# BOpermanis/SP-SLAM

Hardware: AMD Instinct MI355X
Metric: RGB-D frames/sec (track+planes+poseOpt) at 640x480; ATE vs CPU ref (higher is better)
Workload: dtype u8+f32+f64

## Files before the change

### include/spslam_gpu.h

```cpp
#ifndef SPSLAM_GPU_H
#define SPSLAM_GPU_H

#include <stddef.h>
#include <stdint.h>

#ifdef __cplusplus
extern "C" {
#endif

#define SPSLAM_OK 0
#define SPSLAM_ERR_ARG (-1)
#define SPSLAM_ERR_CAPACITY (-2)
#define SPSLAM_ERR_HIP (-3)
#define SPSLAM_ERR_NOT_READY (-4)

typedef struct spslam_ctx spslam_ctx;

typedef struct spslam_keypoint {
    float x, y;
    float size;
    float angle;
    float response;
    int32_t octave;
    int32_t class_id;
} spslam_keypoint;

typedef struct spslam_orb_params {
    int nfeatures;
    float scale_factor;
    int nlevels;
    int ini_th_fast;
    int min_th_fast;
    int width, height;
    int max_batch;
} spslam_orb_params;

#define SPSLAM_MAX_LEVELS 8

int spslam_create(int device, const spslam_orb_params* params, spslam_ctx** out);
void spslam_destroy(spslam_ctx* ctx);
const char* spslam_last_error(const spslam_ctx* ctx);

int spslam_orb_tables(const spslam_ctx* ctx, int* nlevels, float* scale, float* inv_scale, float* sigma2,
                      float* inv_sigma2, int* features_per_level);

int spslam_orb_max_keypoints(const spslam_ctx* ctx);

int spslam_orb_extract(spslam_ctx* ctx, const uint8_t* gray, int w, int h, int stride, spslam_keypoint* kps,
                       uint8_t* desc, int cap, int* n);

int spslam_orb_extract_batch_device(spslam_ctx* ctx, const uint8_t* d_gray, int n_frames, size_t frame_stride,
                                    int stride, spslam_keypoint* d_kps, uint8_t* d_desc, int* d_counts,
                                    int cap_per_frame, void* hip_stream);

int spslam_orb_debug_stage(spslam_ctx* ctx, int frame, int level, int stage, void* out, int cap, int* n);
int spslam_orb_level_size(const spslam_ctx* ctx, int level, int* w, int* h);

typedef struct spslam_point_obs {
    float u, v;
    float ur;
    float inv_sigma2;
    float xw[3];
    int32_t kp_index;
} spslam_point_obs;

#define SPSLAM_PLANE_EDGE 0
#define SPSLAM_PARALLEL_EDGE 1
#define SPSLAM_VERTICAL_EDGE 2

typedef struct spslam_plane_obs {
    float meas[4];
    float world[4];
    int32_t kind;
    int32_t plane_index;
    int32_t map_plane_id;
    int32_t pad;
} spslam_plane_obs;

typedef struct spslam_plane_config {
    double angle_info, distance_info, parallel_info, vertical_info, chi, vp_chi;
} spslam_plane_config;

typedef struct spslam_pose_problem {
    float Tcw[16];
    float fx, fy, cx, cy, bf;
    int32_t n_points;
    int32_t n_planes;
    int32_t point_offset;
    int32_t plane_offset;
    int32_t pad;
} spslam_pose_problem;

typedef struct spslam_pose_result {
    float Tcw[16];
    int32_t n_inliers;
    int32_t lm_iterations;
    int32_t trial_passes;
    int32_t trials;
} spslam_pose_result;

int spslam_pose_optimize(spslam_ctx* ctx, const spslam_pose_problem* problem, const spslam_point_obs* points,
                         const spslam_plane_obs* planes, const spslam_plane_config* cfg, spslam_pose_result* result,
                         uint8_t* point_outlier, uint8_t* plane_outlier);

int spslam_pose_optimize_batch_device(spslam_ctx* ctx, int n, const spslam_pose_problem* d_problems,
                                      const spslam_point_obs* d_points, const spslam_plane_obs* d_planes,
                                      const spslam_plane_config* cfg, const spslam_pose_result* d_init_from,
                                      spslam_pose_result* d_results, uint8_t* d_point_outlier,
                                      uint8_t* d_plane_outlier, void* hip_stream);

typedef struct spslam_lba_keyframe {
    float Tcw[16];
    float fx, fy, cx, cy, bf;
    int32_t id;
    int32_t fixed;
    int32_t pad;
} spslam_lba_keyframe;

typedef struct spslam_lba_point {
    float xw[3];
    int32_t id;
    int32_t obs_offset;
    int32_t n_obs;
} spslam_lba_point;

typedef struct spslam_lba_point_obs {
    int32_t kf;
    float u, v;
    float ur;
    float inv_sigma2;
} spslam_lba_point_obs;

typedef struct spslam_lba_plane {
    float world[4];
    int32_t id;
    int32_t obs_offset;
    int32_t n_obs;
    int32_t pad;
} spslam_lba_plane;

typedef struct spslam_lba_plane_obs {
    int32_t kf;
    int32_t kind;
    float meas[4];
} spslam_lba_plane_obs;

typedef struct spslam_lba_problem {
    int32_t n_kf, n_points, n_planes;
    int32_t kf_offset, point_offset, plane_offset;
    int32_t n_point_obs, n_plane_obs;
} spslam_lba_problem;

typedef struct spslam_lba_result {
    int32_t iterations[2];
    int32_t n_point_outliers;
    int32_t n_plane_outliers;
    int32_t status;
    int32_t trials;
    int32_t stopped;
    int32_t pad;
    float phase_us[8];
} spslam_lba_result;

int spslam_lba_optimize(spslam_ctx* ctx, const spslam_lba_problem* problem, const spslam_lba_keyframe* kfs,
                        const spslam_lba_point* points, const spslam_lba_point_obs* point_obs,
                        const spslam_lba_plane* planes, const spslam_lba_plane_obs* plane_obs,
                        const spslam_plane_config* cfg, float* kf_out, float* pt_out, float* pl_out,
                        uint8_t* point_obs_outlier, uint8_t* plane_obs_outlier, spslam_lba_result* result,
                        const volatile uint8_t* stop_flag);

#define SPSLAM_LBA_G2O_ORDER 0
#define SPSLAM_LBA_FAST_ORDER 1
int spslam_lba_set_order(spslam_ctx* ctx, int order);

int spslam_lba_debug_stop_after(spslam_ctx* ctx, int trials);

int spslam_lba_set_team(spslam_ctx* ctx, int workgroups);

int spslam_lba_optimize_batch_device(spslam_ctx* ctx, int n, const spslam_lba_problem* problems,
                                     const spslam_lba_problem* d_problems, const spslam_lba_keyframe* d_kfs,
                                     const spslam_lba_point* d_points, const spslam_lba_point_obs* d_point_obs,
                                     const spslam_lba_plane* d_planes, const spslam_lba_plane_obs* d_plane_obs,
                                     const spslam_plane_config* cfg, float* d_kf_out, float* d_pt_out,
                                     float* d_pl_out, uint8_t* d_point_obs_outlier, uint8_t* d_plane_obs_outlier,
                                     spslam_lba_result* d_results, const int32_t* d_stop_flags, void* hip_stream);

typedef struct spslam_plane_params {
    int cloud_dis;
    int min_size;
    float angle_threshold;
    float distance_threshold;
    float fx, fy, cx, cy;
    int width, height;
    double line_ratio;
    float line_distance_threshold;
    float image_bounds[4];
} spslam_plane_params;

typedef struct spslam_plane {
    float coef[4];
    int32_t n_inliers;
    int32_t inlier_offset;
    int32_t n_contour;
    int32_t contour_offset;
} spslam_plane;

int spslam_planes_configure(spslam_ctx* ctx, const spslam_plane_params* params);

int spslam_planes_capacity(const spslam_ctx* ctx, int* planes_cap, int* inlier_cap, int* contour_cap);

int spslam_planes_extract(spslam_ctx* ctx, const float* depth, int w, int h, int stride_floats,
                          spslam_plane* planes, int planes_cap, int* n_planes, int32_t* inliers, int32_t* contours);

int spslam_planes_extract_batch_device(spslam_ctx* ctx, const float* d_depth, int n_frames, size_t frame_stride,
                                       int stride_floats, spslam_plane* d_planes, int* d_counts,
                                       int32_t* d_inliers, int32_t* d_contours, void* hip_stream);

typedef struct spslam_supposed_plane {
    float coef[4];
    float line[6];
    int32_t source_plane;
    int32_t n_line;
    int32_t line_offset;
    int32_t n_patch;
    int32_t patch_offset;
    int32_t pad;
} spslam_supposed_plane;

int spslam_supposed_capacity(const spslam_ctx* ctx, int* supp_cap, int* line_cap, int* patch_points);

int spslam_planes_generate_from_boundaries(spslam_ctx* ctx, const float* depth, int w, int h, int stride_floats,
                                           spslam_supposed_plane* out, int cap, int* n, int32_t* line_idx,
                                           float* patch_xyz);

int spslam_planes_generate_from_boundaries_batch_device(spslam_ctx* ctx, const float* d_depth, int n_frames,
                                                        size_t frame_stride, int stride_floats,
                                                        const spslam_plane* d_planes, const int* d_counts,
                                                        const int32_t* d_contours, spslam_supposed_plane* d_out,
                                                        int* d_out_counts, int32_t* d_line_idx, float* d_patch,
                                                        void* hip_stream);

int spslam_planes_select_cloud_set(spslam_ctx* ctx, int set);

typedef struct spslam_line_candidate {
    float line[6];
    int32_t n_inliers;
    int32_t iterations;
    int32_t flags;
    int32_t idx_offset;
} spslam_line_candidate;
int spslam_supposed_debug(spslam_ctx* ctx, int frame, int plane, spslam_line_candidate* cand, int* n_cand,
                          int32_t* idx, int idx_cap);

int spslam_planes_debug(spslam_ctx* ctx, int frame, int what, void* out, int* n_points);

int spslam_debug_plane_labels(spslam_ctx* ctx, int keep);

int spslam_debug_plane_not_seen(spslam_ctx* ctx, const float* planes, int n_planes, const float* coefs, int n_coefs,
                                int* not_seen);

int spslam_debug_libm64(spslam_ctx* ctx, int kind, const double* a, const double* b, int n, double* out);

int spslam_debug_pose_spin_cap(spslam_ctx* ctx, int cap);

int spslam_debug_force_solve_failures(spslam_ctx* ctx, unsigned trial_mask);

#define SPSLAM_GRID_COLS 64
#define SPSLAM_GRID_ROWS 48

typedef struct spslam_frame_params {
    float fx, fy, cx, cy;
    float dist[5];
    float bf;
    int width, height;
} spslam_frame_params;

int spslam_frame_configure(spslam_ctx* ctx, const spslam_frame_params* params, float* bounds, float* grid_inv);

int spslam_frame_rgbd(spslam_ctx* ctx, const spslam_keypoint* kps, int n, const float* depth, int w, int h,
                      int stride_floats, spslam_keypoint* keys_un, float* mv_depth, float* mv_uright,
                      int32_t* grid_off, int32_t* grid_idx);

int spslam_frame_rgbd_batch_device(spslam_ctx* ctx, const spslam_keypoint* d_kps, const int* d_counts,
                                   int cap_per_frame, const float* d_depth, int n_frames, size_t frame_stride,
                                   int stride_floats, spslam_keypoint* d_keys_un, float* d_mv_depth,
                                   float* d_mv_uright, int32_t* d_grid_off, int32_t* d_grid_idx,
                                   int* d_plane_counts, int* d_supp_counts, void* hip_stream);

typedef struct spslam_map_plane {
    float world[4];
    int32_t id;
    int32_t boundary_offset;
    int32_t n_boundary;
    int32_t pad;
} spslam_map_plane;

typedef struct spslam_assoc_params {
    float dis_th;
    float angle_th;
    float ver_th;
    float par_th;
} spslam_assoc_params;

typedef struct spslam_assoc_frame {
    float Tcw[16];
    int32_t map_offset;
    int32_t n_map;
    int32_t carry;
    int32_t pad;
} spslam_assoc_frame;

int spslam_planes_associate(spslam_ctx* ctx, const spslam_assoc_frame* frame, const float* coefs, int n_planes,
                            const spslam_map_plane* map_planes, int n_map, const float* boundary_xyz,
                            int n_boundary, const spslam_assoc_params* params, int32_t* match, int32_t* parallel,
                            int32_t* vertical, int* new_plane);

int spslam_planes_associate_batch_device(spslam_ctx* ctx, int n_frames, const spslam_assoc_frame* d_frames,
                                         const void* d_planes_a, int stride_a, const int* d_count_a, int cap_a,
                                         const void* d_planes_b, int stride_b, const int* d_count_b, int cap_b,
                                         const spslam_map_plane* d_map, const float* d_boundary_xyz, int max_map,
                                         const spslam_assoc_params* params, int32_t* d_match, int32_t* d_parallel,
                                         int32_t* d_vertical, int* d_new_plane, void* hip_stream);

typedef struct spslam_proj_point {
    float xw[3];
    float angle;
    int32_t octave;
    int32_t n_obs;
    int32_t last_index;
    int32_t id;
    uint8_t desc[32];
} spslam_proj_point;

typedef struct spslam_proj_frame {
    float Tcw[16];
    float Tlw[16];
    int32_t point_offset;
    int32_t n_points;
    int32_t pad[2];
} spslam_proj_frame;

typedef struct spslam_match_params {
    float th;
    int32_t mono;
    int32_t check_orientation;
    int32_t retry_below;
} spslam_match_params;

int spslam_search_by_projection(spslam_ctx* ctx, const spslam_proj_frame* frame, const spslam_proj_point* points,
                                const spslam_keypoint* keys_un, const uint8_t* desc, const float* uright, int n_kp,
                                const int32_t* grid_off, const int32_t* grid_idx, const spslam_match_params* params,
                                int32_t* match, int* nmatches);

int spslam_search_by_projection_batch_device(spslam_ctx* ctx, int n_frames, const spslam_proj_frame* d_frames,
                                             const spslam_proj_point* d_points, int max_points,
                                             const spslam_keypoint* d_keys_un, const uint8_t* d_desc,
                                             const float* d_uright, const int32_t* d_grid_off,
                                             const int32_t* d_grid_idx, const int* d_counts, int cap,
                                             const spslam_match_params* params, int32_t* d_match, int* d_nmatches,
                                             void* hip_stream);

typedef struct spslam_local_point {
    float xw[3];
    float normal[3];
    float min_dist;
    float max_dist;
    int32_t id;
    int32_t n_obs;
    int32_t pad[2];
    uint8_t desc[32];
} spslam_local_point;

typedef struct spslam_local_frame {
    float Tcw[16];
    int32_t point_offset;
    int32_t n_points;
    int32_t seen_offset;
    int32_t stamp;
} spslam_local_frame;

typedef struct spslam_local_params {
    float th;
    float nn_ratio;
    float view_cos_limit;
    int32_t pad;
} spslam_local_params;

int spslam_search_local_points(spslam_ctx* ctx, const spslam_local_frame* frame, const spslam_local_point* points,
                               const spslam_keypoint* keys_un, const uint8_t* desc, const float* uright, int n_kp,
                               const int32_t* grid_off, const int32_t* grid_idx, const uint8_t* taken,
                               const spslam_local_params* params, int32_t* match, int* nmatches, uint8_t* in_view);

int spslam_search_local_points_batch_device(spslam_ctx* ctx, int n_frames, const spslam_local_frame* d_frames,
                                            const spslam_local_point* d_points, int max_points,
                                            const spslam_keypoint* d_keys_un, const uint8_t* d_desc,
                                            const float* d_uright, const int32_t* d_grid_off,
                                            const int32_t* d_grid_idx, const int* d_counts, int cap,
                                            const uint8_t* d_taken, const spslam_local_params* params,
                                            int32_t* d_match, int* d_nmatches, uint8_t* d_in_view,
                                            const int32_t* d_seen, void* hip_stream);

typedef struct spslam_grab_params {
    int32_t channels;
    int32_t rgb;
    int32_t depth_u16;
    float depth_scale;
} spslam_grab_params;

int spslam_grab_rgbd(spslam_ctx* ctx, const uint8_t* color, int color_stride, const void* depth, int depth_stride,
                     int w, int h, const spslam_grab_params* params, uint8_t* gray, float* depth_out);

int spslam_grab_rgbd_batch_device(spslam_ctx* ctx, int n_frames, const uint8_t* d_color, size_t color_frame_stride,
                                  int color_stride, const void* d_depth, size_t depth_frame_stride, int depth_stride,
                                  int w, int h, const spslam_grab_params* params, uint8_t* d_gray, float* d_depth_out,
                                  void* hip_stream);

int spslam_grab_fuse_cloud(spslam_ctx* ctx, int enable);

#define SPSLAM_TRACK_MOTION_MODEL 0
#define SPSLAM_TRACK_DISCARD 1
#define SPSLAM_TRACK_LOCAL_MAP 2
#define SPSLAM_TRACK_MOTION_PRIOR 3
#define SPSLAM_TRACK_LAST_FRAME 4

typedef struct spslam_track_batch {
    const spslam_keypoint* keys_un;
    const float* uright;
    const int* kp_counts;
    int32_t cap;
    const spslam_proj_frame* proj_frames;
    const spslam_proj_point* proj_points;
    const int32_t* proj_match;
    spslam_local_frame* local_frames;
    const spslam_local_point* local_points;
    const int32_t* local_match;
    uint8_t* taken;
    const void* planes_a;
    const void* planes_b;
    const int* count_a;
    const int* count_b;
    int32_t stride_a, stride_b, cap_a, cap_b;
    const spslam_map_plane* map;
    const int32_t* assoc_match;
    const int32_t* assoc_parallel;
    const int32_t* assoc_vertical;
    spslam_assoc_frame* assoc_frames_next;
    const uint8_t* plane_outlier;
    int32_t* next_match;
    int32_t* next_parallel;
    int32_t* next_vertical;
    spslam_assoc_frame* assoc_frames_first;
    int32_t* seen;
    spslam_proj_frame* next_frames;
    spslam_proj_point* next_points;
    float* velocity;
    const uint8_t* point_outlier_local;
    spslam_pose_problem* problems;
    spslam_point_obs* points;
    spslam_plane_obs* planes;
    int32_t* edge_of_kp;
    const spslam_pose_result* results;
    const uint8_t* point_outlier;
    float fx, fy, cx, cy, bf;
    int32_t pad;
} spslam_track_batch;

int spslam_track_graph_batch_device(spslam_ctx* ctx, int n_frames, int stage, const spslam_track_batch* batch,
                                    void* hip_stream);

#define SPSLAM_REFKF_PREPARE 0
#define SPSLAM_REFKF_SELECT 1

typedef struct spslam_refkf_batch {
    const int32_t* nmatches;
    uint8_t* fallback;
    int32_t* refkf_counts;
    const int32_t* bow_nmatches;
    const int32_t* bow_match;
    const int32_t* refkf_rows;
    const int32_t* refkf_index;
    int32_t rows_stride, pad;
    const int32_t* refkf_sets;
    const spslam_assoc_frame* assoc_frames;
    uint8_t* apply;
    int8_t* state;
    int32_t* refkf_match;
    spslam_proj_frame* refkf_frames;
    spslam_assoc_frame* refkf_assoc;
} spslam_refkf_batch;

int spslam_track_refkf_batch_device(spslam_ctx* ctx, int n_frames, int stage, const spslam_track_batch* mm,
                                    const spslam_refkf_batch* rk, void* hip_stream);

typedef struct spslam_refkf_vote {
    const int32_t* kf_base;
    const int32_t* kf_sets;
    int32_t ids_per_kf;
    int32_t n_kf;
    int32_t new_kf;
    int32_t pad;
    const int8_t* state;
    int32_t* refkf_index;
    int32_t* refkf_sets;
    int32_t* refkf_pairs;
} spslam_refkf_vote;

int spslam_track_refkf_vote_batch_device(spslam_ctx* ctx, int n_frames, const spslam_track_batch* mm,
                                         const spslam_refkf_vote* vote, void* hip_stream);

typedef struct spslam_frame_region {
    void* dst;
    const void* src;
    int64_t frame_bytes;
    int64_t dst_stride;
    int64_t src_stride;
} spslam_frame_region;

int spslam_masked_frame_copy_device(spslam_ctx* ctx, int n_frames, const uint8_t* flags, int n_regions,
                                    const spslam_frame_region* regions, void* hip_stream);

typedef struct spslam_bow_params {
    float nn_ratio;
    int32_t check_orientation;
} spslam_bow_params;

int spslam_bow_load_vocabulary(spslam_ctx* ctx, const char* text, size_t len, int* k, int* L, int* n_nodes,
                               int* n_words);

int spslam_bow_transform(spslam_ctx* ctx, const uint8_t* desc, int n, int levelsup, uint32_t* bow_words,
                         double* bow_values, int* n_bow, uint32_t* fv_nodes, int32_t* fv_start,
                         int32_t* fv_features, int* n_fv);

int spslam_bow_transform_batch_device(spslam_ctx* ctx, int n_frames, const uint8_t* d_desc, const int* d_counts,
                                      int cap, int levelsup, uint32_t* d_bow_words, double* d_bow_values,
                                      int* d_n_bow, uint32_t* d_fv_nodes, int32_t* d_fv_start,
                                      int32_t* d_fv_features, int* d_n_fv, void* hip_stream);

typedef struct spslam_bow_side {
    const uint8_t* desc;
    const spslam_keypoint* keys;
    const uint8_t* has_point;
    const int* counts;
    const uint32_t* fv_nodes;
    const int32_t* fv_start;
    const int32_t* fv_features;
    const int* n_fv;
    int32_t cap;
    int32_t pad;
} spslam_bow_side;

int spslam_search_by_bow(spslam_ctx* ctx, const uint8_t* kf_desc, const spslam_keypoint* kf_keys,
                         const uint8_t* kf_has_point, int kf_n, const uint32_t* kf_fv_nodes,
                         const int32_t* kf_fv_start, const int32_t* kf_fv_features, int kf_n_fv,
                         const uint8_t* f_desc, const spslam_keypoint* f_keys, int f_n, const uint32_t* f_fv_nodes,
                         const int32_t* f_fv_start, const int32_t* f_fv_features, int f_n_fv,
                         const spslam_bow_params* params, int32_t* match, int* nmatches);

int spslam_search_by_bow_batch_device(spslam_ctx* ctx, int n_pairs, const int32_t* d_pairs,
                                      const spslam_bow_side* keyframe, const spslam_bow_side* frame,
                                      const spslam_bow_params* params, int32_t* d_match, int* d_nmatches,
                                      void* hip_stream);

typedef struct spslam_step_config {
    int32_t n_frames, width, height, kp_cap;
    int32_t pipelined, tail_priority, orb_priority, planes_priority;
    spslam_grab_params grab;
    spslam_match_params match;
    spslam_local_params local;
    spslam_assoc_params assoc;
    spslam_plane_config pose;
    float fx, fy, cx, cy, bf;
    int32_t pad;
} spslam_step_config;

typedef struct spslam_step_frames {
    const uint8_t* color;
    size_t color_frame_stride;
    const void* depth;
    size_t depth_frame_stride;
    int32_t color_stride, depth_stride;
} spslam_step_frames;

typedef struct spslam_step_tracking {
    const spslam_proj_frame* proj_frames;
    const spslam_proj_point* proj_points;
    spslam_local_frame* local_frames;
    const spslam_local_point* local_points;
    const spslam_assoc_frame* assoc_frames1;
    spslam_assoc_frame* assoc_frames2;
    const spslam_map_plane* map;
    const float* boundary_xyz;
    int32_t max_proj_points, max_local_points, max_map, pad;
} spslam_step_tracking;

typedef struct spslam_step_set {
    uint8_t* gray;
    float* depth;
    spslam_keypoint* kps;
    uint8_t* desc;
    int* counts;
    spslam_plane* planes;
    int* plane_counts;
    int32_t* inliers;
    int32_t* contours;
    spslam_supposed_plane* supposed;
    int* supposed_counts;
    int32_t* lines;
    float* patch;
} spslam_step_set;

typedef struct spslam_step_tail {
    spslam_keypoint* keys_un;
    float* mv_depth;
    float* uright;
    int32_t* grid_off;
    int32_t* grid_idx;
    int32_t* match;
    int* nmatches;
    uint8_t* taken;
    int32_t* local_match;
    int* local_nmatches;
    int32_t* edge_of_kp;
    int32_t* assoc[2][3];
    int* new_plane[2];
    spslam_pose_problem* problems[2];
    spslam_point_obs* points[2];
    spslam_plane_obs* planes[2];
    uint8_t* point_outlier[2];
    uint8_t* plane_outlier[2];
    spslam_pose_result* results[2];
} spslam_step_tail;

typedef struct spslam_step spslam_step;
int spslam_step_create(spslam_ctx* ctx, const spslam_step_config* cfg, const spslam_step_set* sets ,
                       const spslam_step_tail* tail , spslam_step** out);
int spslam_step_buffers(const spslam_step* step, spslam_step_set* sets , spslam_step_tail* tail);
int spslam_step_prime(spslam_step* step, const spslam_step_frames* first);
int spslam_step_run(spslam_step* step, const spslam_step_frames* next, const spslam_step_tracking* tracking);
int spslam_step_sync(spslam_step* step);
void* spslam_step_stream(const spslam_step* step);
void spslam_step_destroy(spslam_step* step);

int spslam_set_timing(spslam_ctx* ctx, int enable);
int spslam_kernel_times(spslam_ctx* ctx, double* total_ms, long long* launches, int max_kinds);
const char* spslam_kernel_name(int kind);

#ifdef __cplusplus
}
#endif

#endif
```

### sp-slam_amd/csrc/capi_ctx.h

```cpp
#pragma once
#include <hip/hip_runtime.h>

#include <algorithm>
#include <cstdint>
#include <cstdio>
#include <cstdlib>
#include <initializer_list>
#include <string>
#include <vector>

#include "../../include/spslam_gpu.h"
#include "orb_launch.h"
#include "plane_launch.h"
#include "pose_launch.h"
#include "supposed_launch.h"
#include "frame_launch.h"
#include "lba_launch.h"
#include "assoc_launch.h"
#include "bow_launch.h"
#include "match_launch.h"
#include "track_launch.h"
#include "grab_launch.h"

using namespace spslam;

struct EventTimer : KernelTimer {
    struct Pair { int kind; hipEvent_t e0, e1; };
    std::vector<Pair> pending;
    std::vector<hipEvent_t> pool;
    double total_ms[kNumKernelKinds] = {};
    long long count[kNumKernelKinds] = {};
    hipEvent_t cur[kNumKernelKinds] = {};
    hipEvent_t get() {
        if (!pool.empty()) { hipEvent_t e = pool.back(); pool.pop_back(); return e; }
        hipEvent_t e = nullptr;
        (void)hipEventCreate(&e);
        return e;
    }
    void begin(int kind, hipStream_t s) override { cur[kind] = get(); (void)hipEventRecord(cur[kind], s); }
    void end(int kind, hipStream_t s) override {
        hipEvent_t e1 = get();
        (void)hipEventRecord(e1, s);
        pending.push_back(Pair{kind, cur[kind], e1});
    }
    void collect() {
        for (auto& p : pending) {
            float ms = 0.f;
            if (hipEventSynchronize(p.e1) == hipSuccess && hipEventElapsedTime(&ms, p.e0, p.e1) == hipSuccess) {
                total_ms[p.kind] += ms;
                count[p.kind] += 1;
            }
            pool.push_back(p.e0);
            pool.push_back(p.e1);
        }
        pending.clear();
    }
    void reset() { collect(); for (int k = 0; k < kNumKernelKinds; k++) { total_ms[k] = 0; count[k] = 0; } }
    ~EventTimer() override {
        for (auto& p : pending) { (void)hipEventDestroy(p.e0); (void)hipEventDestroy(p.e1); }
        for (auto e : pool) (void)hipEventDestroy(e);
    }
};

template <class T = uint8_t>
struct DevBuf {
    T* p = nullptr;
    size_t cap = 0;
    DevBuf() = default;
    DevBuf(const DevBuf&) = delete;
    DevBuf& operator=(const DevBuf&) = delete;
    ~DevBuf() { release(); }
    operator T*() const { return p; }
    void release() {
        if (p) (void)hipFree(p);
        p = nullptr;
        cap = 0;
    }
    hipError_t alloc(size_t bytes) {
        release();
        const hipError_t e = hipMalloc((void**)&p, bytes);
        if (e == hipSuccess) cap = bytes; else p = nullptr;
        return e;
    }
    hipError_t reserve(size_t bytes, hipStream_t s) {
        if (bytes <= cap) return hipSuccess;
        const hipError_t e = hipStreamSynchronize(s);
        return e != hipSuccess ? e : alloc(bytes);
    }
};

struct CtxStreams {
    hipStream_t stream = nullptr;
    hipStream_t orb_aux = nullptr;
    hipEvent_t orb_fork = nullptr, orb_join = nullptr;
    hipEvent_t lba_done = nullptr;
    int32_t* h_lba_stop = nullptr;
    int32_t* d_lba_stop = nullptr;
    CtxStreams() = default;
    CtxStreams(const CtxStreams&) = delete;
    CtxStreams& operator=(const CtxStreams&) = delete;
    ~CtxStreams() {
        if (lba_done) (void)hipEventDestroy(lba_done);
        if (h_lba_stop) (void)hipHostFree(h_lba_stop);
        if (orb_fork) (void)hipEventDestroy(orb_fork);
        if (orb_join) (void)hipEventDestroy(orb_join);
        if (orb_aux) (void)hipStreamDestroy(orb_aux);
        if (stream) (void)hipStreamDestroy(stream);
    }
};

struct spslam_ctx : CtxStreams {
    int device = 0;
    int num_cus = 256;
    spslam_orb_params p{};
    std::string err;
    std::vector<float> scale, inv_scale, sigma2, inv_sigma2;
    std::vector<int> nfeat;
    int umax[16]{};
    OrbGeom geom{};
    long long pyr_frame_stride = 0, blur_frame_stride = 0;
    int max_kp = 0;
    DevBuf<> d_pyr, d_blur, d_score;
    OrbBuffers b{};
    DevBuf<uint32_t> d_cand, d_keys;
    DevBuf<uint16_t> d_cand_cnt, d_keynode;
    DevBuf<LevelKp> d_lvl_kp;
    DevBuf<int> d_lvl_cnt;
    DevBuf<> d_in;
    DevBuf<spslam_keypoint> d_kps;
    DevBuf<> d_desc;
    DevBuf<int> d_cnt;
    const uint8_t* last_gray = nullptr;
    size_t last_frame_stride = 0;
    int last_stride = 0, last_frames = 0;
    EventTimer* timer = nullptr;
    DevBuf<> d_pose_scratch;
    bool planes_ready = false;
    PlaneGeom pg{};
    PlaneBuffers pb{};
    float* plane_cloud[2] = {nullptr, nullptr};
    int cloud_set = 0;
    struct CloudTag { const float* depth = nullptr; int n = 0; } cloud_tag[2];
    bool grab_cloud = [] { const char* e = getenv("SPSLAM_GRAB_CLOUD"); return e && e[0] == '1'; }();
    DevBuf<> d_plane_scratch;
    DevBuf<float> d_depth_in;
    DevBuf<spslam_plane> d_planes1;
    DevBuf<int> d_plane_cnt1;
    DevBuf<int32_t> d_inl1, d_con1;
    int plane_last_frames = 0;
    SuppParams sp{};
    SuppBuffers sb{};
    DevBuf<> d_supp_scratch;
    DevBuf<spslam_supposed_plane> d_supp1;
    DevBuf<int> d_supp_cnt1;
    DevBuf<int32_t> d_line1;
    DevBuf<float> d_patch1;
    int supp_last_frames = 0;
    bool frame_ready = false;
    FrameGeom fg{};
    DevBuf<> d_frame1;
    DevBuf<> d_lba_scratch;
    DevBuf<long long> d_lba_off;
    int lba_stop_after = -1;
    int lba_order = SPSLAM_LBA_G2O_ORDER;
    int lba_team = 0;
    DevBuf<int> d_lba_ctl;
    int pose_spin_cap = 0;
    unsigned solve_fail_mask = 0;
    DevBuf<> d_lba_stage;
    DevBuf<int2> d_lba_work;
    DevBuf<float> d_assoc_dist;
    DevBuf<> d_match_scratch;
    DevBuf<> d_vocab;
    VocabDev vocab{};
    DevBuf<> d_bow_scratch;
    DevBuf<> d_bow_stage;

    ~spslam_ctx() {
        if (lba_done) (void)hipEventSynchronize(lba_done);
        delete timer;
    }
};

inline int fail(spslam_ctx* c, int code, const char* fmt, const char* what = "") {
    if (c) {
        char buf[512];
        std::snprintf(buf, sizeof buf, fmt, what);
        c->err = buf;
    }
    return code;
}
#define HIP_CHECK(ctx, expr)                                                                  \
    do {                                                                                      \
        hipError_t e_ = (expr);                                                               \
        if (e_ != hipSuccess) return fail(ctx, SPSLAM_ERR_HIP, #expr ": %s", hipGetErrorString(e_)); \
    } while (0)

struct StageSlot {
    const void* src;
    size_t upload, bytes;
    StageSlot(const void* s, size_t up, size_t b) : src(s), upload(up), bytes(b) {}
    StageSlot(const void* s, size_t b) : StageSlot(s, b, b) {}
    StageSlot(size_t b) : StageSlot(nullptr, 0, b) {}
};

inline size_t stage_layout(const StageSlot* slots, int n, size_t* off) {
    size_t bytes = 0;
    for (int i = 0; i < n; i++) { off[i] = bytes; bytes += (slots[i].bytes + 255) / 256 * 256; }
    return bytes;
}

struct Stage {
    static constexpr int kMaxSlots = 18;
    spslam_ctx* c;
    uint8_t* q = nullptr;
    bool temporary = false;
    size_t off[kMaxSlots] = {};
    explicit Stage(spslam_ctx* ctx) : c(ctx) {}
    Stage(const Stage&) = delete;
    Stage& operator=(const Stage&) = delete;
    ~Stage() { if (temporary && q) (void)hipFreeAsync(q, c->stream); }
    int open(std::initializer_list<StageSlot> slots, DevBuf<>* persistent = nullptr, size_t grow = 1) {
        const int n = (int)slots.size();
        if (n > kMaxSlots) return fail(c, SPSLAM_ERR_ARG, "too many staging slots%s", "");
        const size_t bytes = stage_layout(slots.begin(), n, off);
        if (!persistent) {
            HIP_CHECK(c, hipMallocAsync((void**)&q, bytes, c->stream));
            temporary = true;
        } else {
            if (bytes > persistent->cap) HIP_CHECK(c, persistent->reserve(bytes * grow, c->stream));
            q = *persistent;
        }
        for (int i = 0; i < n; i++) {
            const StageSlot& s = slots.begin()[i];
            if (s.upload) HIP_CHECK(c, hipMemcpyAsync(q + off[i], s.src, s.upload, hipMemcpyHostToDevice, c->stream));
        }
        return SPSLAM_OK;
    }
    template <class T>
    T* slot(int i) const { return (T*)(q + off[i]); }
    int close() {
        uint8_t* t = temporary ? q : nullptr;
        q = nullptr;
        if (t) HIP_CHECK(c, hipFreeAsync(t, c->stream));
        return SPSLAM_OK;
    }
};
```

### sp-slam_amd/csrc/capi_planes.cpp

```cpp
#include "capi_ctx.h"

#include <cmath>
#include <cstring>
#include <random>

namespace {

hipError_t configure_supposed(spslam_ctx* c, const spslam_plane_params* p) {
    const PlaneGeom& g = c->pg;
    SuppParams& sp = c->sp;
    sp.line_ratio = p->line_ratio;
    const double T = (double)p->line_distance_threshold * (double)p->line_distance_threshold;
    float f = (float)T;
    while ((double)f >= T && f > 0.f) f = std::nextafter(f, 0.f);
    while ((double)std::nextafter(f, 1.f) < T) f = std::nextafter(f, 1.f);
    sp.sqr_th_f = f;
    const bool nob = p->image_bounds[0] == 0.f && p->image_bounds[1] == 0.f && p->image_bounds[2] == 0.f &&
                     p->image_bounds[3] == 0.f;
    sp.min_x = nob ? 0.f : p->image_bounds[0];
    sp.max_x = nob ? (float)p->width : p->image_bounds[1];
    sp.min_y = nob ? 0.f : p->image_bounds[2];
    sp.max_y = nob ? (float)p->height : p->image_bounds[3];
    sp.supp_cap = kMaxSuppPerFrame;
    sp.line_cap = g.contour_cap;
    int ns = 0;
    for (float v = -0.25f; v < 0.25f; v = (float)((double)v + 0.01)) {
        if (ns >= kMaxPatchSteps) return hipErrorInvalidValue;
        sp.steps[ns++] = v;
    }
    sp.n_steps = ns;
    const size_t F = (size_t)c->p.max_batch, CC = (size_t)g.contour_cap;
    SuppBuffers& b = c->sb;
    const size_t bytes = (size_t)kSuppRndTable * 4 +
                         F * kMaxPlanesPerFrame * kMaxLinesPerBoundary * sizeof(LineCand) +
                         F * kMaxPlanesPerFrame * sizeof(int) + F * CC * (4 + 16 + 4 + 1) +
                         F * kMaxPlanesPerFrame * 8 * sizeof(long long) + 9 * 256;
    hipError_t e = c->d_supp_scratch.alloc(bytes);
    if (e != hipSuccess) return e;
    uint8_t* q = c->d_supp_scratch;
    auto carve = [&](size_t n) { uint8_t* r = q; q += (n + 255) / 256 * 256; return r; };
    b.rnd = (const uint32_t*)carve((size_t)kSuppRndTable * 4);
    b.cand = (LineCand*)carve(F * kMaxPlanesPerFrame * kMaxLinesPerBoundary * sizeof(LineCand));
    b.n_cand = (int*)carve(F * kMaxPlanesPerFrame * sizeof(int));
    b.line_idx = (int32_t*)carve(F * CC * 4);
    b.big = (float4*)carve(F * CC * 16);
    b.big_sh = (int*)carve(F * CC * 4);
    b.big_flag = (uint8_t*)carve(F * CC);
    b.prof = (long long*)carve(F * kMaxPlanesPerFrame * 8 * sizeof(long long));
    e = hipMemset(b.prof, 0, F * kMaxPlanesPerFrame * 8 * sizeof(long long));
    if (e != hipSuccess) return e;
    std::vector<uint32_t> tab(kSuppRndTable);
    std::mt19937 mt(12345u);
    for (auto& v : tab) v = (uint32_t)mt() >> 1;
    e = hipMemcpy((void*)b.rnd, tab.data(), tab.size() * 4, hipMemcpyHostToDevice);
    if (e != hipSuccess) return e;
    const size_t patch = (size_t)sp.n_steps * sp.n_steps;
    if ((e = c->d_supp1.alloc(sp.supp_cap * sizeof(spslam_supposed_plane))) != hipSuccess) return e;
    if ((e = c->d_supp_cnt1.alloc(16)) != hipSuccess) return e;
    if ((e = c->d_line1.alloc(CC * 4)) != hipSuccess) return e;
    return c->d_patch1.alloc(sp.supp_cap * patch * 12);
}

}

extern "C" {

int spslam_planes_configure(spslam_ctx* c, const spslam_plane_params* p) {
    if (!c || !p) return SPSLAM_ERR_ARG;
    if (p->cloud_dis < 1 || p->width < 1 || p->height < 1 || p->fx == 0.f || p->fy == 0.f)
        return fail(c, SPSLAM_ERR_ARG, "bad plane parameters%s", "");
    HIP_CHECK(c, hipSetDevice(c->device));
    HIP_CHECK(c, hipStreamSynchronize(c->stream));
    PlaneGeom& g = c->pg;
    g.w = p->width;
    g.h = p->height;
    g.ds = p->cloud_dis;
    g.W = (int)std::ceil(p->width / (float)p->cloud_dis);
    g.H = (int)std::ceil(p->height / (float)p->cloud_dis);
    g.N = g.W * g.H;
    if (g.H > 512) return fail(c, SPSLAM_ERR_ARG, "organized cloud taller than 512 rows%s", "");
    if (g.N > 160000) return fail(c, SPSLAM_ERR_ARG, "organized cloud larger than the LDS state map%s", "");
    if (3 * 10 * g.W * 4 > 65536) return fail(c, SPSLAM_ERR_ARG, "organized cloud wider than the LDS row band%s", "");
    g.fx = p->fx; g.fy = p->fy; g.cx = p->cx; g.cy = p->cy;
    g.min_size = p->min_size;
    g.ang_cos = std::cos((float)(0.017453 * p->angle_threshold));
    g.dist_th = p->distance_threshold;
    g.inlier_cap = g.N;
    g.contour_cap = 4 * g.N;
    const long long N = g.N, F = c->p.max_batch, IWH = (long long)(g.W + 1) * (g.H + 1);
    PlaneBuffers& b = c->pb;
    c->planes_ready = false;
    c->plane_last_frames = c->supp_last_frames = 0;
    c->plane_cloud[0] = c->plane_cloud[1] = nullptr;
    c->sb = SuppBuffers{};
    const int keep_labels = b.keep_labels;
    b = PlaneBuffers{};
    b.keep_labels = keep_labels;
    const long long SH = wave_size(g.W, g.H);
    b.cloud_fs = 3 * N; b.wave_fs = SH; b.dist_fs = N; b.integral_fs = 6 * (IWH + g.W + 1); b.normal_fs = 3 * N; b.pd_fs = N;
    b.labels_fs = N; b.work_fs = 4 * N; b.grown_fs = N; b.maps_fs = 2 * N;
    const size_t bytes = F * (sizeof(float) * (2 * b.cloud_fs + b.wave_fs + b.dist_fs + b.normal_fs + b.pd_fs) +
                              sizeof(double) * b.integral_fs + sizeof(uint32_t) * b.labels_fs +
                              sizeof(int) * (b.work_fs + b.grown_fs) + b.maps_fs + 16 * sizeof(long long)) + 8192;
    HIP_CHECK(c, c->d_plane_scratch.alloc(bytes));
    uint8_t* q = c->d_plane_scratch;
    auto carve = [&](size_t n) { uint8_t* r = q; q += (n + 255) / 256 * 256; return r; };
    b.integral = (double*)carve(F * b.integral_fs * sizeof(double));
    c->plane_cloud[0] = (float*)carve(F * b.cloud_fs * 4);
    c->plane_cloud[1] = (float*)carve(F * b.cloud_fs * 4);
    b.cloud = c->plane_cloud[0];
    c->cloud_set = 0;
    c->cloud_tag[0] = c->cloud_tag[1] = {};
    b.wave = (float*)carve(F * b.wave_fs * 4);
    b.dist = (float*)carve(F * b.dist_fs * 4);
    b.normal = (float*)carve(F * b.normal_fs * 4);
    b.pd = (float*)carve(F * b.pd_fs * 4);
    b.labels = (uint32_t*)carve(F * b.labels_fs * 4);
    b.work = (int*)carve(F * b.work_fs * 4);
    b.grown = (int*)carve(F * b.grown_fs * 4);
    b.maps = (uint8_t*)carve(F * b.maps_fs);
    b.ts = (long long*)carve(F * 16 * sizeof(long long));
    HIP_CHECK(c, c->d_depth_in.alloc((size_t)g.w * g.h * sizeof(float)));
    HIP_CHECK(c, c->d_planes1.alloc(kMaxPlanesPerFrame * sizeof(spslam_plane)));
    HIP_CHECK(c, c->d_plane_cnt1.alloc(16));
    HIP_CHECK(c, c->d_inl1.alloc((size_t)g.inlier_cap * 4));
    HIP_CHECK(c, c->d_con1.alloc((size_t)g.contour_cap * 4));
    HIP_CHECK(c, configure_supposed(c, p));
    c->planes_ready = true;
    return SPSLAM_OK;
}

int spslam_planes_capacity(const spslam_ctx* c, int* planes_cap, int* inlier_cap, int* contour_cap) {
    if (!c || !c->planes_ready) return SPSLAM_ERR_NOT_READY;
    if (planes_cap) *planes_cap = kMaxPlanesPerFrame;
    if (inlier_cap) *inlier_cap = c->pg.inlier_cap;
    if (contour_cap) *contour_cap = c->pg.contour_cap;
    return SPSLAM_OK;
}

int spslam_planes_extract_batch_device(spslam_ctx* c, const float* d_depth, int n_frames, size_t frame_stride,
                                       int stride_floats, spslam_plane* d_planes, int* d_counts,
                                       int32_t* d_inliers, int32_t* d_contours, void* hip_stream) {
    if (!c) return SPSLAM_ERR_ARG;
    if (!c->planes_ready) return fail(c, SPSLAM_ERR_NOT_READY, "spslam_planes_configure not called%s", "");
    if (!d_depth || !d_planes || !d_counts || !d_inliers || !d_contours || n_frames < 1 ||
        n_frames > c->p.max_batch || stride_floats < c->pg.w)
        return fail(c, SPSLAM_ERR_ARG, "bad argument%s", " to spslam_planes_extract_batch_device");
    HIP_CHECK(c, hipSetDevice(c->device));
    hipStream_t s = (hipStream_t)hip_stream;
    auto& tag = c->cloud_tag[c->cloud_set];
    const bool have_cloud = tag.depth == d_depth && n_frames <= tag.n &&
                            frame_stride == (size_t)c->pg.w * c->pg.h && stride_floats == c->pg.w;
    tag = {};
    HIP_CHECK(c, plane_launch(c->pg, c->pb, n_frames, d_depth, (long long)frame_stride, stride_floats, d_planes,
                              d_counts, kMaxPlanesPerFrame, d_inliers, d_contours, s, c->timer, have_cloud));
    c->plane_last_frames = n_frames;
    return SPSLAM_OK;
}

int spslam_planes_extract(spslam_ctx* c, const float* depth, int w, int h, int stride_floats, spslam_plane* planes,
                          int planes_cap, int* n_planes, int32_t* inliers, int32_t* contours) {
    if (!c || !n_planes) return SPSLAM_ERR_ARG;
    if (!c->planes_ready) return fail(c, SPSLAM_ERR_NOT_READY, "spslam_planes_configure not called%s", "");
    if (!depth || w != c->pg.w || h != c->pg.h || stride_floats < w)
        return fail(c, SPSLAM_ERR_ARG, "depth size does not match the plane configuration%s", "");
    HIP_CHECK(c, hipSetDevice(c->device));
    HIP_CHECK(c, hipMemcpy2DAsync(c->d_depth_in, (size_t)w * 4, depth, (size_t)stride_floats * 4, (size_t)w * 4, h,
                                  hipMemcpyHostToDevice, c->stream));
    int rc = spslam_planes_extract_batch_device(c, c->d_depth_in, 1, (size_t)w * h, w, c->d_planes1, c->d_plane_cnt1,
                                                c->d_inl1, c->d_con1, c->stream);
    if (rc) return rc;
    int n = 0;
    spslam_plane tmp[kMaxPlanesPerFrame];
    HIP_CHECK(c, hipMemcpyAsync(&n, c->d_plane_cnt1, sizeof(int), hipMemcpyDeviceToHost, c->stream));
    HIP_CHECK(c, hipMemcpyAsync(tmp, c->d_planes1, sizeof tmp, hipMemcpyDeviceToHost, c->stream));
    HIP_CHECK(c, hipStreamSynchronize(c->stream));
    *n_planes = n;
    if (n > planes_cap) return fail(c, SPSLAM_ERR_CAPACITY, "plane buffer too small%s", "");
    int ni = 0, nc = 0;
    for (int k = 0; k < n; k++) {
        planes[k] = tmp[k];
        ni = std::max(ni, tmp[k].inlier_offset + tmp[k].n_inliers);
        nc = std::max(nc, tmp[k].contour_offset + tmp[k].n_contour);
    }
    if (inliers && ni) HIP_CHECK(c, hipMemcpy(inliers, c->d_inl1, (size_t)ni * 4, hipMemcpyDeviceToHost));
    if (contours && nc) HIP_CHECK(c, hipMemcpy(contours, c->d_con1, (size_t)nc * 4, hipMemcpyDeviceToHost));
    return SPSLAM_OK;
}

int spslam_supposed_capacity(const spslam_ctx* c, int* supp_cap, int* line_cap, int* patch_points) {
    if (!c || !c->planes_ready) return SPSLAM_ERR_NOT_READY;
    if (supp_cap) *supp_cap = c->sp.supp_cap;
    if (line_cap) *line_cap = c->sp.line_cap;
    if (patch_points) *patch_points = c->sp.n_steps * c->sp.n_steps;
    return SPSLAM_OK;
}

int spslam_planes_select_cloud_set(spslam_ctx* c, int set) {
    if (!c) return SPSLAM_ERR_ARG;
    if (!c->planes_ready) return fail(c, SPSLAM_ERR_NOT_READY, "spslam_planes_configure not called%s", "");
    if (set < 0 || set > 1) return fail(c, SPSLAM_ERR_ARG, "cloud set not 0 or 1%s", "");
    c->pb.cloud = c->plane_cloud[set];
    c->cloud_set = set;
    return SPSLAM_OK;
}

int spslam_planes_generate_from_boundaries_batch_device(spslam_ctx* c, const float* d_depth, int n_frames,
                                                        size_t frame_stride, int stride_floats,
                                                        const spslam_plane* d_planes, const int* d_counts,
                                                        const int32_t* d_contours, spslam_supposed_plane* d_out,
                                                        int* d_out_counts, int32_t* d_line_idx, float* d_patch,
                                                        void* hip_stream) {
    if (!c) return SPSLAM_ERR_ARG;
    if (!c->planes_ready) return fail(c, SPSLAM_ERR_NOT_READY, "spslam_planes_configure not called%s", "");
    if (!d_depth || !d_planes || !d_counts || !d_contours || !d_out || !d_out_counts || !d_line_idx || !d_patch ||
        n_frames < 1 || stride_floats < c->pg.w)
        return fail(c, SPSLAM_ERR_ARG, "bad argument%s", " to spslam_planes_generate_from_boundaries_batch_device");
    if (n_frames > c->plane_last_frames)
        return fail(c, SPSLAM_ERR_NOT_READY, "%s", "more frames than the last plane extraction holds");
    HIP_CHECK(c, hipSetDevice(c->device));
    hipStream_t s = (hipStream_t)hip_stream;
    HIP_CHECK(c, supp_launch(c->pg, c->pb, c->sp, c->sb, n_frames, d_depth, (long long)frame_stride, stride_floats,
                             d_planes, d_counts, d_contours, d_out, d_out_counts, d_line_idx, d_patch, s, c->timer));
    c->supp_last_frames = n_frames;
    return SPSLAM_OK;
}

int spslam_planes_generate_from_boundaries(spslam_ctx* c, const float* depth, int w, int h, int stride_floats,
                                           spslam_supposed_plane* out, int cap, int* n, int32_t* line_idx,
                                           float* patch_xyz) {
    if (!c || !n) return SPSLAM_ERR_ARG;
    if (!c->planes_ready) return fail(c, SPSLAM_ERR_NOT_READY, "spslam_planes_configure not called%s", "");
    if (!depth || w != c->pg.w || h != c->pg.h || stride_floats < w)
        return fail(c, SPSLAM_ERR_ARG, "depth size does not match the plane configuration%s", "");
    if (c->plane_last_frames < 1) return fail(c, SPSLAM_ERR_NOT_READY, "%s", "spslam_planes_extract not called");
    HIP_CHECK(c, hipSetDevice(c->device));
    HIP_CHECK(c, hipMemcpy2DAsync(c->d_depth_in, (size_t)w * 4, depth, (size_t)stride_floats * 4, (size_t)w * 4, h,
                                  hipMemcpyHostToDevice, c->stream));
    int rc = spslam_planes_generate_from_boundaries_batch_device(c, c->d_depth_in, 1, (size_t)w * h, w, c->d_planes1,
                                                                 c->d_plane_cnt1, c->d_con1, c->d_supp1,
                                                                 c->d_supp_cnt1, c->d_line1, c->d_patch1, c->stream);
    if (rc) return rc;
    int m = 0;
    std::vector<spslam_supposed_plane> tmp(c->sp.supp_cap);
    HIP_CHECK(c, hipMemcpyAsync(&m, c->d_supp_cnt1, sizeof(int), hipMemcpyDeviceToHost, c->stream));
    HIP_CHECK(c, hipMemcpyAsync(tmp.data(), c->d_supp1, tmp.size() * sizeof(spslam_supposed_plane),
                                hipMemcpyDeviceToHost, c->stream));
    HIP_CHECK(c, hipStreamSynchronize(c->stream));
    *n = m;
    const int stored = std::min(m, c->sp.supp_cap);
    if (m > cap || m > c->sp.supp_cap) return fail(c, SPSLAM_ERR_CAPACITY, "supposed-plane buffer too small%s", "");
    int nl = 0;
    for (int k = 0; k < stored; k++) {
        out[k] = tmp[k];
        nl = std::max(nl, tmp[k].line_offset + tmp[k].n_line);
    }
    const size_t patch = (size_t)c->sp.n_steps * c->sp.n_steps;
    if (line_idx && nl) HIP_CHECK(c, hipMemcpy(line_idx, c->d_line1, (size_t)nl * 4, hipMemcpyDeviceToHost));
    if (patch_xyz && stored)
        HIP_CHECK(c, hipMemcpy(patch_xyz, c->d_patch1, stored * patch * 12, hipMemcpyDeviceToHost));
    return SPSLAM_OK;
}

int spslam_planes_associate_batch_device(spslam_ctx* c, int n_frames, const spslam_assoc_frame* d_frames,
                                         const void* d_planes_a, int stride_a, const int* d_count_a, int cap_a,
                                         const void* d_planes_b, int stride_b, const int* d_count_b, int cap_b,
                                         const spslam_map_plane* d_map, const float* d_boundary_xyz, int max_map,
                                         const spslam_assoc_params* params, int32_t* d_match, int32_t* d_parallel,
                                         int32_t* d_vertical, int* d_new_plane, void* hip_stream) {
    if (!c) return SPSLAM_ERR_ARG;
    if (n_frames < 1 || !d_frames || !params || !d_match || !d_parallel || !d_vertical || max_map < 0 ||
        (cap_a > 0 && (!d_planes_a || !d_count_a || stride_a < 16)) || cap_a < 0 || cap_b < 0 ||
        (cap_b > 0 && (!d_planes_b || !d_count_b || stride_b < 16)) || (max_map > 0 && (!d_map || !d_boundary_xyz)))
        return fail(c, SPSLAM_ERR_ARG, "bad argument%s", " to spslam_planes_associate_batch_device");
    HIP_CHECK(c, hipSetDevice(c->device));
    hipStream_t s = (hipStream_t)hip_stream;
    const size_t need = std::max<size_t>((size_t)n_frames * (cap_a + cap_b) * max_map * sizeof(float), 256);
    HIP_CHECK(c, c->d_assoc_dist.reserve(need, s));
    AssocSources S{(const uint8_t*)d_planes_a, cap_b > 0 ? (const uint8_t*)d_planes_b : nullptr, stride_a,
                   stride_b, d_count_a, cap_b > 0 ? d_count_b : nullptr, cap_a, cap_b};
    HIP_CHECK(c, assoc_launch(n_frames, d_frames, S, d_map, d_boundary_xyz, max_map, *params, c->d_assoc_dist,
                              d_match, d_parallel, d_vertical, d_new_plane, s, c->timer));
    return SPSLAM_OK;
}

int spslam_planes_associate(spslam_ctx* c, const spslam_assoc_frame* frame, const float* coefs, int n_planes,
                            const spslam_map_plane* map_planes, int n_map, const float* boundary_xyz,
                            int n_boundary, const spslam_assoc_params* params, int32_t* match, int32_t* parallel,
                            int32_t* vertical, int* new_plane) {
    if (!c || !frame || !params || n_planes < 0 || n_map < 0 || n_boundary < 0 ||
        (n_planes && (!coefs || !match || !parallel || !vertical)) || (n_map && !map_planes) ||
        (n_boundary && !boundary_xyz))
        return SPSLAM_ERR_ARG;
    for (int j = 0; j < n_map; j++)
        if (map_planes[j].n_boundary < 0 || map_planes[j].boundary_offset < 0 ||
            (long long)map_planes[j].boundary_offset + map_planes[j].n_boundary > n_boundary)
            return fail(c, SPSLAM_ERR_ARG, "map plane boundary range outside the boundary array%s", "");
    HIP_CHECK(c, hipSetDevice(c->device));
    spslam_assoc_frame F = *frame;
    F.map_offset = 0;
    F.n_map = n_map;
    const int cap = std::max(n_planes, 1);
    Stage st(c);
    if (int rc = st.open({{&F, sizeof F}, {coefs, (size_t)n_planes * 16, (size_t)cap * 16}, {&n_planes, sizeof(int)},
                           {map_planes, n_map * sizeof(spslam_map_plane), std::max(n_map, 1) * sizeof(spslam_map_plane)},
                           {boundary_xyz, (size_t)n_boundary * 12, (size_t)std::max(n_boundary, 1) * 12},
                           (size_t)cap * 4 * 3, sizeof(int)}))
        return rc;
    auto* d_out = st.slot<int32_t>(5);
    if (F.carry && n_planes) {
        HIP_CHECK(c, hipMemcpyAsync(d_out, match, (size_t)n_planes * 4, hipMemcpyHostToDevice, c->stream));
        HIP_CHECK(c, hipMemcpyAsync(d_out + cap, parallel, (size_t)n_planes * 4, hipMemcpyHostToDevice, c->stream));
        HIP_CHECK(c, hipMemcpyAsync(d_out + 2 * cap, vertical, (size_t)n_planes * 4, hipMemcpyHostToDevice, c->stream));
    }
    int rc = spslam_planes_associate_batch_device(
        c, 1, st.slot<spslam_assoc_frame>(0), st.slot<void>(1), 16, st.slot<int>(2), cap, nullptr, 0, nullptr, 0,
        st.slot<spslam_map_plane>(3), st.slot<float>(4), n_map, params, d_out, d_out + cap, d_out + 2 * cap,
        st.slot<int>(6), c->stream);
    if (rc) return rc;
    int np = 0;
    if (n_planes) {
        HIP_CHECK(c, hipMemcpyAsync(match, d_out, (size_t)n_planes * 4, hipMemcpyDeviceToHost, c->stream));
        HIP_CHECK(c, hipMemcpyAsync(parallel, d_out + cap, (size_t)n_planes * 4, hipMemcpyDeviceToHost, c->stream));
        HIP_CHECK(c, hipMemcpyAsync(vertical, d_out + 2 * cap, (size_t)n_planes * 4, hipMemcpyDeviceToHost, c->stream));
    }
    HIP_CHECK(c, hipMemcpyAsync(&np, st.slot<int>(6), sizeof(int), hipMemcpyDeviceToHost, c->stream));
    if ((rc = st.close())) return rc;
    HIP_CHECK(c, hipStreamSynchronize(c->stream));
    if (new_plane) *new_plane = np;
    return SPSLAM_OK;
}

int spslam_debug_plane_not_seen(spslam_ctx* c, const float* planes, int n_planes, const float* coefs, int n_coefs,
                                int* not_seen) {
    if (!c || n_planes < 0 || n_coefs < 0 || (n_planes && !planes) || (n_coefs && (!coefs || !not_seen)))
        return SPSLAM_ERR_ARG;
    if (!n_coefs) return SPSLAM_OK;
    HIP_CHECK(c, hipSetDevice(c->device));
    const size_t cb = (size_t)n_coefs * 16;
    Stage st(c);
    if (int rc = st.open({{planes, (size_t)n_planes * 16, (size_t)std::max(n_planes, 1) * 16}, {coefs, cb},
                          (size_t)n_coefs * 4}))
        return rc;
    HIP_CHECK(c, plane_not_seen_debug_launch(st.slot<float>(0), n_planes, st.slot<float>(1), n_coefs,
                                             st.slot<int>(2), c->stream));
    HIP_CHECK(c, hipMemcpyAsync(not_seen, st.slot<int>(2), (size_t)n_coefs * 4, hipMemcpyDeviceToHost, c->stream));
    if (int rc = st.close()) return rc;
    HIP_CHECK(c, hipStreamSynchronize(c->stream));
    return SPSLAM_OK;
}

int spslam_debug_plane_labels(spslam_ctx* c, int keep) {
    if (!c) return SPSLAM_ERR_ARG;
    c->pb.keep_labels = keep ? 1 : 0;
    return SPSLAM_OK;
}

int spslam_supposed_debug(spslam_ctx* c, int frame, int plane, spslam_line_candidate* cand, int* n_cand,
                          int32_t* idx, int idx_cap) {
    static_assert(sizeof(spslam_line_candidate) == sizeof(LineCand), "candidate layout");
    if (!c || !cand || !n_cand) return SPSLAM_ERR_ARG;
    if (frame < 0 || frame >= c->supp_last_frames || plane < 0 || plane >= kMaxPlanesPerFrame)
        return fail(c, SPSLAM_ERR_NOT_READY, "no supposed-plane data for that frame%s", "");
    HIP_CHECK(c, hipSetDevice(c->device));
    HIP_CHECK(c, hipDeviceSynchronize());
    int nc = 0;
    HIP_CHECK(c, hipMemcpy(&nc, c->sb.n_cand + frame * kMaxPlanesPerFrame + plane, sizeof(int), hipMemcpyDeviceToHost));
    nc = std::min(std::max(nc, 0), kMaxLinesPerBoundary);
    LineCand lc[kMaxLinesPerBoundary];
    if (nc)
        HIP_CHECK(c, hipMemcpy(lc, c->sb.cand + ((size_t)frame * kMaxPlanesPerFrame + plane) * kMaxLinesPerBoundary,
                               nc * sizeof(LineCand), hipMemcpyDeviceToHost));
    *n_cand = nc;
    int lo = 0;
    for (int k = 0; k < nc; k++) {
        std::memcpy(&cand[k], &lc[k], sizeof(LineCand));
        if (lc[k].flags & 1) {
            const int m = lc[k].n_inliers;
            if (idx && lo + m <= idx_cap && m)
                HIP_CHECK(c, hipMemcpy(idx + lo, c->sb.line_idx + (size_t)frame * c->pg.contour_cap + lc[k].idx_off,
                                       (size_t)m * 4, hipMemcpyDeviceToHost));
            cand[k].idx_offset = lo;
            lo += m;
        } else {
            cand[k].idx_offset = -1;
        }
    }
    return lo > idx_cap ? SPSLAM_ERR_CAPACITY : SPSLAM_OK;
}

int spslam_planes_debug(spslam_ctx* c, int frame, int what, void* out, int* n_points) {
    if (!c || !out) return SPSLAM_ERR_ARG;
    if (!c->planes_ready || frame < 0 || frame >= c->plane_last_frames)
        return fail(c, SPSLAM_ERR_NOT_READY, "no plane data for that frame%s", "");
    HIP_CHECK(c, hipSetDevice(c->device));
    HIP_CHECK(c, hipDeviceSynchronize());
    const PlaneBuffers& b = c->pb;
    const long long N = c->pg.N;
    if (n_points) *n_points = (int)N;
    if (what == 0 || what == 1) {
        const float* src = what == 0 ? b.cloud + frame * b.cloud_fs : b.normal + frame * b.normal_fs;
        std::vector<float> soa(3 * N);
        HIP_CHECK(c, hipMemcpy(soa.data(), src, 3 * N * 4, hipMemcpyDeviceToHost));
        float* o = (float*)out;
        for (long long i = 0; i < N; i++) { o[3 * i] = soa[i]; o[3 * i + 1] = soa[N + i]; o[3 * i + 2] = soa[2 * N + i]; }
        return SPSLAM_OK;
    }
    if (what == 2) {
        HIP_CHECK(c, hipMemcpy(out, b.dist + frame * b.dist_fs, N * 4, hipMemcpyDeviceToHost));
        return SPSLAM_OK;
    }
    if (what == 3) {
        bool in_lds = false;
        plane_segment_lds_bytes(c->pg, &in_lds);
        if (in_lds && !b.keep_labels)
            return fail(c, SPSLAM_ERR_NOT_READY, "labels are kept only after spslam_debug_plane_labels(ctx, 1)%s", "");
        HIP_CHECK(c, hipMemcpy(out, b.labels + frame * b.labels_fs, N * 4, hipMemcpyDeviceToHost));
        return SPSLAM_OK;
    }
    if (what == 4) {
        HIP_CHECK(c, hipMemcpy(out, b.ts + frame * 16, 16 * sizeof(long long), hipMemcpyDeviceToHost));
        return SPSLAM_OK;
    }
    if (what == 5) {
        HIP_CHECK(c, hipMemcpy(out, c->sb.prof + (size_t)frame * kMaxPlanesPerFrame * 8,
                               kMaxPlanesPerFrame * 8 * sizeof(long long), hipMemcpyDeviceToHost));
        return SPSLAM_OK;
    }
    return fail(c, SPSLAM_ERR_ARG, "unknown debug stage%s", "");
}

}
```

### sp-slam_amd/csrc/supposed_kernels.hip

```cpp
#include <cfloat>

#include "libm_restated.h"
#include "plane_not_seen.h"
#include "supposed_launch.h"

namespace spslam {
namespace supp {

constexpr int kThreads = 256, kWaves = 4;
constexpr int kMaxWaves = 8;
constexpr int kBatch = 64;
constexpr int kLdsPts = 2048;
constexpr int kMaxTrials = 1001;

#ifdef SPSLAM_SUPP_PROF
#define SUPP_CLK() ((long long)__builtin_amdgcn_s_memrealtime())
#define SUPP_T(k) do { if (t == 0) { const long long c_ = SUPP_CLK(); pr[k] += c_ - pt; pt = c_; } } while (0)
#else
#define SUPP_T(k) do { } while (0)
#endif

struct Shared {
    int s0[kBatch], s1[kBatch], cnt[kBatch];
    int nb, fail, done, have;
    int iterations, best, best_s0, best_s1;
    double k;
    float line[6];
    float acc[9];
    int red[kMaxWaves];
    int n_inl, flags;
    int s0x[kBatch], s1x[kBatch], nbb[2], failb[2];
};

__device__ __forceinline__ int wave_sum(int v) {
#pragma unroll
    for (int o = 32; o > 0; o >>= 1) v += __shfl_xor(v, o);
    return v;
}
template <int NT>
__device__ int block_sum(int v, Shared& S) {
    const int lane = threadIdx.x & 63, wave = threadIdx.x >> 6;
    v = wave_sum(v);
    __syncthreads();
    if (lane == 0) S.red[wave] = v;
    __syncthreads();
    int s = 0;
#pragma unroll
    for (int w = 0; w < NT / 64; w++) s += S.red[w];
    return s;
}

__device__ __forceinline__ void line_from_samples(const float4 a, const float4 b, float* c) {
    c[0] = a.x; c[1] = a.y; c[2] = a.z;
    float d0 = b.x - a.x, d1 = b.y - a.y, d2 = b.z - a.z;
    const float sq = d0 * d0 + d1 * d1 + d2 * d2;
    if (sq > 0.f) {
        const float s = sqrtf(sq);
        d0 /= s; d1 /= s; d2 /= s;
    }
    c[3] = d0; c[4] = d1; c[5] = d2;
}
__device__ __forceinline__ void normalize4(float* d) {
    const float sq = (d[0] * d[0] + d[2] * d[2]) + (d[1] * d[1] + 0.f);
    if (sq > 0.f) {
        const float s = sqrtf(sq);
        d[0] /= s; d[1] /= s; d[2] /= s;
    }
}
__device__ __forceinline__ float line_sqd(const float* lp, const float* ld, const float4 p) {
    const float ax = lp[0] - p.x, ay = lp[1] - p.y, az = lp[2] - p.z;
    const float cx = ay * ld[2] - az * ld[1];
    const float cy = az * ld[0] - ax * ld[2];
    const float cz = ax * ld[1] - ay * ld[0];
    return (cx * cx + cz * cz) + (cy * cy + 0.f);
}

__device__ void roots2(float b, float c, float* r) {
    r[0] = 0.f;
    float d = (float)(b * b - 4.0 * c);
    if (d < 0.0) d = 0.0;
    const float sd = sqrtf(d);
    r[2] = 0.5f * (b + sd);
    r[1] = 0.5f * (b - sd);
}
__device__ void roots3(const float (&m)[3][3], float* r) {
    const float c0 = m[0][0] * m[1][1] * m[2][2] + 2.f * m[0][1] * m[0][2] * m[1][2] - m[0][0] * m[1][2] * m[1][2] -
                     m[1][1] * m[0][2] * m[0][2] - m[2][2] * m[0][1] * m[0][1];
    const float c1 = m[0][0] * m[1][1] - m[0][1] * m[0][1] + m[0][0] * m[2][2] - m[0][2] * m[0][2] +
                     m[1][1] * m[2][2] - m[1][2] * m[1][2];
    const float c2 = m[0][0] + m[1][1] + m[2][2];
    if (fabsf(c0) < FLT_EPSILON) { roots2(c2, c1, r); return; }
    const float s_inv3 = (float)(1.0 / 3.0), s_sqrt3 = sqrtf(3.0f);
    const float c2_over_3 = c2 * s_inv3;
    float a_over_3 = (c1 - c2 * c2_over_3) * s_inv3;
    if (a_over_3 > 0.f) a_over_3 = 0.f;
    const float half_b = 0.5f * (c0 + c2_over_3 * (2.f * c2_over_3 * c2_over_3 - c1));
    float q = half_b * half_b + a_over_3 * a_over_3 * a_over_3;
    if (q > 0.f) q = 0.f;
    const float rho = sqrtf(-a_over_3);
    const float theta = libm::atan2f_(sqrtf(-q), half_b) * s_inv3;
    float st, ct;
    libm::sincosf_(theta, &st, &ct);
    r[0] = c2_over_3 + 2.f * rho * ct;
    r[1] = c2_over_3 - rho * (ct + s_sqrt3 * st);
    r[2] = c2_over_3 - rho * (ct - s_sqrt3 * st);
    float t;
    if (r[0] >= r[1]) { t = r[0]; r[0] = r[1]; r[1] = t; }
    if (r[1] >= r[2]) {
        t = r[1]; r[1] = r[2]; r[2] = t;
        if (r[0] >= r[1]) { t = r[0]; r[0] = r[1]; r[1] = t; }
    }
    if (r[0] <= 0) roots2(c2, c1, r);
}
__device__ float max_abs3(const float (&m)[3][3]) {
    float s = 0.f;
    for (int i = 0; i < 3; i++)
        for (int j = 0; j < 3; j++) s = fmaxf(s, fabsf(m[i][j]));
    if (s <= FLT_MIN) s = 1.f;
    return s;
}
__device__ void line_direction(const float (&cov)[3][3], float* evec) {
    const float scale = max_abs3(cov);
    float s[3][3];
    for (int i = 0; i < 3; i++)
        for (int j = 0; j < 3; j++) s[i][j] = cov[i][j] / scale;
    float r[3];
    roots3(s, r);
    const float eval2 = r[2] * scale;
    const float scale2 = max_abs3(cov);
    for (int i = 0; i < 3; i++)
        for (int j = 0; j < 3; j++) s[i][j] = cov[i][j] / scale2;
    const float sub = eval2 / scale2;
    for (int i = 0; i < 3; i++) s[i][i] -= sub;
    const int pr[3][2] = {{0, 1}, {0, 2}, {1, 2}};
    float v[3][3], len[3];
    for (int k = 0; k < 3; k++) {
        const float* a = s[pr[k][0]];
        const float* b = s[pr[k][1]];
        v[k][0] = a[1] * b[2] - a[2] * b[1];
        v[k][1] = a[2] * b[0] - a[0] * b[2];
        v[k][2] = a[0] * b[1] - a[1] * b[0];
        len[k] = v[k][0] * v[k][0] + v[k][1] * v[k][1] + v[k][2] * v[k][2];
    }
    int k = 2;
    if (len[0] >= len[1] && len[0] >= len[2]) k = 0;
    else if (len[1] >= len[0] && len[1] >= len[2]) k = 1;
    const float sl = sqrtf(len[k]);
    for (int j = 0; j < 3; j++) evec[j] = v[k][j] / sl;
}

struct Cam { float fx, fy, cx, cy, min_x, max_x, min_y, max_y; int w, h, stride; };

__device__ bool is_border_point(const float4 p, const float* __restrict__ depth, const Cam& K) {
    if (p.z < 0.0f) return false;
    const float invz = 1.0f / p.z;
    const float u = fmaf(K.fx * p.x, invz, K.cx);
    const float v = fmaf(K.fy * p.y, invz, K.cy);
    if (isnan(u) || isnan(v)) return true;
    if (!(fabsf(u) < 1e6f) || !(fabsf(v) < 1e6f)) return false;
    const int total = K.w * K.h;
    auto offset = [&](int i, int j) -> int {
        if ((unsigned)i < (unsigned)K.w && (unsigned)j < (unsigned)K.h) return j * K.stride + i;
        const int fi = j * K.w + i;
        return (fi >= 0 && fi < total) ? (fi / K.w) * K.stride + fi % K.w : -1;
    };
    int num = 0, nan = 0;
    float res = 0.f;
    constexpr int kRow = 22;
    const int i0 = (int)(u - 10.f);
    for (int j = (int)(v - 10.f); (float)j < v + 10.f; ++j) {
        float dv[kRow];
#pragma unroll
        for (int k = 0; k < kRow; k++) {
            const int o = offset(i0 + k, j);
            const float x = depth[o < 0 ? 0 : o];
            dv[k] = o < 0 ? 0.f : x;
        }
        int i = i0;
#pragma unroll
        for (int k = 0; k < kRow; k++, ++i) {
            if (!((float)i < u + 10.f)) break;
            const float d = dv[k];
            if ((double)d > 0.05) {
                res += d;
                num++;
            } else if (++nan > 100) {
                return false;
            }
        }
        for (; (float)i < u + 10.f; ++i) {
            const int o = offset(i, j);
            const float d = o < 0 ? 0.f : depth[o];
            if ((double)d > 0.05) {
                res += d;
                num++;
            } else if (++nan > 100) {
                return false;
            }
        }
    }
    if ((double)(p.z - res / (float)num) > 0.1) return false;
    return true;
}

__device__ bool line_in_range(const float* pc, const Cam& K) {
    if (pc[2] < 0.0f) return false;
    const float invz = 1.0f / pc[2];
    const float u = fmaf(K.fx * pc[0], invz, K.cx);
    const float v = fmaf(K.fy * pc[1], invz, K.cy);
    if (u < K.min_x + 50 || u > K.max_x - 50) return false;
    if (v < K.min_y + 50 || v > K.max_y - 50) return false;
    return true;
}

template <int NT>
__device__ int select_within(const float* coef, const float4* Q, uint8_t* flag, int n, float thr, Shared& S) {
    float lp[3] = {coef[0], coef[1], coef[2]}, ld[3] = {coef[3], coef[4], coef[5]};
    normalize4(ld);
    int c = 0;
    for (int i = threadIdx.x; i < n; i += NT) {
        const bool in = line_sqd(lp, ld, Q[i]) <= thr;
        flag[i] = in;
        c += in;
    }
    return block_sum<NT>(c, S);
}

#ifndef SPSLAM_SUPP_OVERLAP
#define SPSLAM_SUPP_OVERLAP 1
#endif
#ifndef SPSLAM_SUPP_OVERLAP_ALL
#define SPSLAM_SUPP_OVERLAP_ALL 0
#endif
#ifndef SPSLAM_SUPP_MINB
#define SPSLAM_SUPP_MINB 3
#endif
template <int NT>
__global__ __launch_bounds__(NT, NT == 256 ? SPSLAM_SUPP_MINB : 1) void supp_lines_kernel(PlaneGeom g, PlaneBuffers pb, SuppParams sp,
                                                              SuppBuffers sb, const float* __restrict__ depth,
                                                              long long depth_fs, int depth_stride,
                                                              const spslam_plane* __restrict__ planes,
                                                              const int* __restrict__ plane_counts,
                                                              const int32_t* __restrict__ contours) {
    __shared__ float4 Qs[kLdsPts];
    __shared__ int shs[kLdsPts];
    __shared__ uint8_t flags_s[kLdsPts];
#ifdef SPSLAM_MEASURE_SKIP_SUPP
    if (g.W > 0) return;
#endif
    __shared__ Shared S;
    constexpr bool kOverlap = SPSLAM_SUPP_OVERLAP && (NT == 512 || SPSLAM_SUPP_OVERLAP_ALL);
    const int f = blockIdx.x, t = threadIdx.x, lane = t & 63, wave = t >> 6;
    const int np = min(plane_counts[f], kMaxPlanesPerFrame);
    const spslam_plane* P = planes + (size_t)f * kMaxPlanesPerFrame;
    const int32_t* con = contours + (size_t)f * g.contour_cap;
    const float* X = pb.cloud + f * pb.cloud_fs;
    const float* Y = X + g.N;
    const float* Z = X + 2 * g.N;
    const Cam K{g.fx, g.fy, g.cx, g.cy, sp.min_x, sp.max_x, sp.min_y, sp.max_y, g.w, g.h, depth_stride};
    const float* D = depth + f * depth_fs;
    const float thr = sp.sqr_th_f;
    for (int q = blockIdx.y; q < np; q += gridDim.y) {
        LineCand* C = sb.cand + ((size_t)f * kMaxPlanesPerFrame + q) * kMaxLinesPerBoundary;
        const int bsize = P[q].n_contour, coff = P[q].contour_offset;
        if (bsize < 50) {
            if (t == 0) sb.n_cand[f * kMaxPlanesPerFrame + q] = 0;
            continue;
        }
        const bool in_lds = bsize <= kLdsPts;
        int32_t* lidx = sb.line_idx + (size_t)f * g.contour_cap + coff;
        auto boundary = [&](float4* Q, int* sh, uint8_t* flag) __attribute__((always_inline)) -> int {
#ifdef SPSLAM_SUPP_PROF
        long long pr[8] = {0, 0, 0, 0, 0, 0, 0, 0}, pt = SUPP_CLK();
#endif
        for (int i = t; i < bsize; i += NT) {
            const int ci = con[coff + i];
            Q[i] = make_float4(X[ci], Y[ci], Z[ci], __int_as_float(ci));
        }
        __syncthreads();
        SUPP_T(0);
        int n = bsize, used = 0, ncand = 0;
        for (int j = 0; j < kMaxLinesPerBoundary; j++) {
            if (t == 0) {
                S.iterations = 0; S.best = -2147483647; S.k = 1.0; S.have = 0; S.done = n < 2;
            }
            if constexpr (kOverlap) {
                if (t < kBatch) S.cnt[t] = 0;
            }
            for (int i = t; i < n; i += NT) sh[i] = i;
            __syncthreads();
            const double one_over_n = 1.0 / (double)n, log_prob = log(1.0 - 0.99);
            int r0 = 0, r1 = 1;
            uint32_t pos = 0;
            int bp0 = 0, bp1 = 0, qh = 0, qn = 0;
            uint64_t gmask = 0;
            uint32_t rnext = wave == 0 ? sb.rnd[lane] : 0u;
            if constexpr (!kOverlap) {
                while (!S.done) {
                    if (wave == 0) {
                        const int it0 = S.iterations;
                        int nb = 0, chk = 0;
                        bool fail = false;
                        while (nb < kBatch && it0 + nb < kMaxTrials) {
                            if (qh == qn) {
                                const uint32_t r = rnext;
                                const uint32_t jv = (lane & 1) ? 1u + r % (uint32_t)(n - 1) : r % (uint32_t)n;
                                pos += 64;
                                rnext = sb.rnd[pos + lane];
    #pragma unroll 4
                                for (int c = 0; c < 32; c++) {
                                    const int j0 = __builtin_amdgcn_readlane((int)jv, 2 * c), j1 = __builtin_amdgcn_readlane((int)jv, 2 * c + 1);
                                    const int i0 = j0 > 1 ? j0 : 0, i1 = j1 > 1 ? j1 : 1;
                                    const int x0 = sh[i0], x1 = sh[i1];
                                    const int a0 = r0, b0 = r1;
                                    const int r1m = j0 == 1 ? a0 : b0;
                                    sh[i0] = a0;
                                    sh[i1] = r1m;
                                    r0 = j0 > 1 ? x0 : (j0 == 1 ? b0 : a0);
                                    r1 = j1 > 1 ? (j1 == j0 ? a0 : x1) : r1m;
                                    bp0 = lane == c ? r0 : bp0;
                                    bp1 = lane == c ? r1 : bp1;
                                }
                                bool good = false;
                                if (lane < 32) {
                                    const float4 a = Q[bp0], b = Q[bp1];
                                    good = a.x != b.x && a.y != b.y && a.z != b.z;
                                }
                                gmask = __ballot(good);
                                qh = 0;
                                qn = 32;
                            }
                            const uint64_t m = gmask & (~0ull << qh) & 0xFFFFFFFFull;
                            if (m == 0) {
                                chk += qn - qh;
                                qh = qn;
                                if (chk >= 1000) { fail = true; break; }
                                continue;
                            }
                            const int gi = __ffsll((unsigned long long)m) - 1;
                            if (chk + (gi - qh) >= 1000) { fail = true; break; }
                            const int s0v = __builtin_amdgcn_readlane(bp0, gi), s1v = __builtin_amdgcn_readlane(bp1, gi);
                            if (lane == 0) { S.s0[nb] = s0v; S.s1[nb] = s1v; }
                            nb++;
                            chk = 0;
                            qh = gi + 1;
                        }
                        if (lane == 0) { S.nb = nb; S.fail = fail; }
                    }
                    __syncthreads();
                    SUPP_T(1);
                    const int nb = S.nb;
                    {
                        constexpr int NW = NT / 64;
                        const int c = wave * (kBatch / NW) + lane / NW, qq = lane % NW;
                        int cnt = 0;
                        if (c < nb) {
                            float L[6];
                            line_from_samples(Q[S.s0[c]], Q[S.s1[c]], L);
                            float ld[3] = {L[3], L[4], L[5]};
                            normalize4(ld);
    #pragma unroll 1
                            for (int i = qq; i < n; i += NW) cnt += line_sqd(L, ld, Q[i]) <= thr;
                        }
    #pragma unroll
                        for (int o = 1; o < NW; o <<= 1) cnt += __shfl_xor(cnt, o);
                        if (qq == 0 && c < nb) S.cnt[c] = cnt;
                    }
                    __syncthreads();
                    SUPP_T(2);
                    if (wave == 0) {
                        const int it0 = S.iterations, best0 = S.best;
                        const double k0 = S.k;
                        const bool act = lane < nb;
                        const int cn = act ? S.cnt[lane] : INT_MIN;
                        int pm = cn, lr;
    #pragma unroll
                        for (int off = 1; off < 64; off <<= 1) {
                            const int y = __shfl_up(pm, off);
                            if (lane >= off) pm = max(pm, y);
                        }
                        int ex = __shfl_up(pm, 1);
                        if (lane == 0) ex = INT_MIN;
                        const bool rec = act && cn > max(ex, best0);
                        double kc = 0.0;
                        if (rec) {
                            const double w = (double)cn * one_over_n;
                            double pno = 1.0 - w * w;
                            pno = fmax(DBL_EPSILON, pno);
                            pno = fmin(1.0 - DBL_EPSILON, pno);
                            kc = log_prob / log(pno);
                        }
                        lr = rec ? lane : -1;
    #pragma unroll
                        for (int off = 1; off < 64; off <<= 1) {
                            const int y = __shfl_up(lr, off);
                            if (lane >= off) lr = max(lr, y);
                        }
                        int lre = __shfl_up(lr, 1);
                        if (lane == 0) lre = -1;
                        const double kb_rec = __shfl(kc, lre < 0 ? 0 : lre);
                        const double kb = lre < 0 ? k0 : kb_rec;
                        const uint64_t m1 = __ballot(act && !((double)(it0 + lane) < kb));
                        const int stop1 = m1 ? __ffsll((unsigned long long)m1) - 1 : 64;
                        const int stop2 = (kMaxTrials - 1) - it0;
                        int proc, it;
                        bool done;
                        if (stop1 < nb && stop1 <= stop2) { proc = stop1; it = it0 + stop1; done = true; }
                        else if (stop2 < nb) { proc = stop2 + 1; it = it0 + stop2 + 1; done = true; }
                        else { proc = nb; it = it0 + nb; done = false; }
                        const uint64_t rm = __ballot(rec) & (proc >= 64 ? ~0ull : ((1ull << proc) - 1ull));
                        double kf = k0;
                        if (rm) {
                            const int L = 63 - __clzll(rm);
                            kf = __shfl(kc, L);
                            if (lane == L) {
                                S.best = cn; S.best_s0 = S.s0[L]; S.best_s1 = S.s1[L]; S.have = 1; S.k = kc;
                            }
                        }
                        if (!done && (S.fail || !((double)it < kf))) done = true;
                        if (lane == 0) {
                            S.iterations = it;
                            S.done = done;
                        }
                    }
                    __syncthreads();
                    SUPP_T(3);
    #ifdef SPSLAM_SUPP_PROF
                    if (t == 0) pr[6]++;
    #endif
                }
            } else {
                auto sample = [&](int sb_, int it0) __attribute__((always_inline)) {
                    int nb = 0, chk = 0;
                    bool fail = false;
                    while (nb < kBatch && it0 + nb < kMaxTrials) {
                        if (qh == qn) {
                            const uint32_t r = rnext;
                            const uint32_t jv = (lane & 1) ? 1u + r % (uint32_t)(n - 1) : r % (uint32_t)n;
                            pos += 64;
                            rnext = sb.rnd[pos + lane];
    #pragma unroll 4
                            for (int c = 0; c < 32; c++) {
                                const int j0 = __builtin_amdgcn_readlane((int)jv, 2 * c), j1 = __builtin_amdgcn_readlane((int)jv, 2 * c + 1);
                                const int i0 = j0 > 1 ? j0 : 0, i1 = j1 > 1 ? j1 : 1;
                                const int x0 = sh[i0], x1 = sh[i1];
                                const int a0 = r0, b0 = r1;
                                const int r1m = j0 == 1 ? a0 : b0;
                                sh[i0] = a0;
                                sh[i1] = r1m;
                                r0 = j0 > 1 ? x0 : (j0 == 1 ? b0 : a0);
                                r1 = j1 > 1 ? (j1 == j0 ? a0 : x1) : r1m;
                                bp0 = lane == c ? r0 : bp0;
                                bp1 = lane == c ? r1 : bp1;
                            }
                            bool good = false;
                            if (lane < 32) {
                                const float4 a = Q[bp0], b = Q[bp1];
                                good = a.x != b.x && a.y != b.y && a.z != b.z;
                            }
                            gmask = __ballot(good);
                            qh = 0;
                            qn = 32;
                        }
                        const uint64_t m = gmask & (~0ull << qh) & 0xFFFFFFFFull;
                        if (m == 0) {
                            chk += qn - qh;
                            qh = qn;
                            if (chk >= 1000) { fail = true; break; }
                            continue;
                        }
                        const int gi = __ffsll((unsigned long long)m) - 1;
                        if (chk + (gi - qh) >= 1000) { fail = true; break; }
                        const int s0v = __builtin_amdgcn_readlane(bp0, gi), s1v = __builtin_amdgcn_readlane(bp1, gi);
                        if (lane == 0) { (sb_ ? S.s0x : S.s0)[nb] = s0v; (sb_ ? S.s1x : S.s1)[nb] = s1v; }
                        nb++;
                        chk = 0;
                        qh = gi + 1;
                    }
                    if (lane == 0) { S.nbb[sb_] = nb; S.failb[sb_] = fail; }
                };
                auto decide = [&](int sb_, int nb) __attribute__((always_inline)) {
                    const int it0 = S.iterations, best0 = S.best;
                    const double k0 = S.k;
                    const bool act = lane < nb;
                    const int cn = act ? S.cnt[lane] : INT_MIN;
                    int pm = cn, lr;
    #pragma unroll
                    for (int off = 1; off < 64; off <<= 1) {
                        const int y = __shfl_up(pm, off);
                        if (lane >= off) pm = max(pm, y);
                    }
                    int ex = __shfl_up(pm, 1);
                    if (lane == 0) ex = INT_MIN;
                    const bool rec = act && cn > max(ex, best0);
                    double kc = 0.0;
                    if (rec) {
                        const double w = (double)cn * one_over_n;
                        double pno = 1.0 - w * w;
                        pno = fmax(DBL_EPSILON, pno);
                        pno = fmin(1.0 - DBL_EPSILON, pno);
                        kc = log_prob / log(pno);
                    }
                    lr = rec ? lane : -1;
    #pragma unroll
                    for (int off = 1; off < 64; off <<= 1) {
                        const int y = __shfl_up(lr, off);
                        if (lane >= off) lr = max(lr, y);
                    }
                    int lre = __shfl_up(lr, 1);
                    if (lane == 0) lre = -1;
                    const double kb_rec = __shfl(kc, lre < 0 ? 0 : lre);
                    const double kb = lre < 0 ? k0 : kb_rec;
                    const uint64_t m1 = __ballot(act && !((double)(it0 + lane) < kb));
                    const int stop1 = m1 ? __ffsll((unsigned long long)m1) - 1 : 64;
                    const int stop2 = (kMaxTrials - 1) - it0;
                    int proc, it;
                    bool done;
                    if (stop1 < nb && stop1 <= stop2) { proc = stop1; it = it0 + stop1; done = true; }
                    else if (stop2 < nb) { proc = stop2 + 1; it = it0 + stop2 + 1; done = true; }
                    else { proc = nb; it = it0 + nb; done = false; }
                    const uint64_t rm = __ballot(rec) & (proc >= 64 ? ~0ull : ((1ull << proc) - 1ull));
                    double kf = k0;
                    if (rm) {
                        const int L = 63 - __clzll(rm);
                        kf = __shfl(kc, L);
                        if (lane == L) {
                            S.best = cn; S.best_s0 = (sb_ ? S.s0x : S.s0)[L]; S.best_s1 = (sb_ ? S.s1x : S.s1)[L];
                            S.have = 1; S.k = kc;
                        }
                    }
                    if (!done && (S.failb[sb_] || !((double)it < kf))) done = true;
                    if (lane == 0) {
                        S.iterations = it;
                        S.done = done;
                    }
                };
                if (wave == 0 && !S.done) sample(0, 0);
                __syncthreads();
                SUPP_T(1);
                int cur = 0;
                while (!S.done) {
                    const int nb = S.nbb[cur];
                    if (wave == 0) {
                        if (!S.failb[cur]) sample(cur ^ 1, S.iterations + nb);
                        else if (lane == 0) { S.nbb[cur ^ 1] = 0; S.failb[cur ^ 1] = 1; }
                    } else {
                        constexpr int LP = NT / 64 - 1;
                        const int u = t - 64, c = u / LP, qq = u - c * LP;
                        if (c < nb) {
                            float L[6];
                            line_from_samples(Q[(cur ? S.s0x : S.s0)[c]], Q[(cur ? S.s1x : S.s1)[c]], L);
                            float ld[3] = {L[3], L[4], L[5]};
                            normalize4(ld);
                            int cnt = 0;
#pragma unroll 1
                            for (int i = qq; i < n; i += LP) cnt += line_sqd(L, ld, Q[i]) <= thr;
                            atomicAdd(&S.cnt[c], cnt);
                        }
                    }
                    __syncthreads();
                    SUPP_T(2);
                    if (wave == 0) {
                        decide(cur, nb);
                        S.cnt[lane] = 0;
                    }
                    __syncthreads();
                    SUPP_T(3);
#ifdef SPSLAM_SUPP_PROF
                    if (t == 0) pr[6]++;
#endif
                    cur ^= 1;
                }
            }
            int n_inl = 0;
            if (S.have) {
                float c0[6];
                line_from_samples(Q[S.best_s0], Q[S.best_s1], c0);
                n_inl = select_within<NT>(c0, Q, flag, n, thr, S);
                if (n_inl > 2) {
                    constexpr int kG = 8;
                    if (wave == 0 && lane < 3) {
                        float s = 0.f;
                        int i = 0;
                        for (; i + kG <= n; i += kG) {
                            float v[kG];
#pragma unroll
                            for (int u = 0; u < kG; u++) {
                                const float4 p = Q[i + u];
                                v[u] = flag[i + u] ? (lane == 0 ? p.x : lane == 1 ? p.y : p.z) : 0.f;
                            }
#pragma unroll
                            for (int u = 0; u < kG; u++) s += v[u];
                        }
                        for (; i < n; i++) {
                            const float4 p = Q[i];
                            s += flag[i] ? (lane == 0 ? p.x : lane == 1 ? p.y : p.z) : 0.f;
                        }
                        S.acc[lane] = s / (float)n_inl;
                    }
                    __syncthreads();
                    if (wave == 0 && lane < 6) {
                        const float cx = S.acc[0], cy = S.acc[1], cz = S.acc[2];
                        auto term = [&](int i) __attribute__((always_inline)) {
                            const float4 p = Q[i];
                            const float x = p.x - cx, y = p.y - cy, z = p.z - cz;
                            const float a = lane == 0 ? y : lane == 1 ? y : lane == 2 ? z : lane == 3 ? x : lane == 4 ? y : z;
                            const float b = lane == 0 ? y : lane == 1 ? z : lane == 2 ? z : x;
                            return flag[i] ? a * b : 0.f;
                        };
                        float s = 0.f;
                        int i = 0;
                        for (; i + kG <= n; i += kG) {
                            float v[kG];
#pragma unroll
                            for (int u = 0; u < kG; u++) v[u] = term(i + u);
#pragma unroll
                            for (int u = 0; u < kG; u++) s += v[u];
                        }
                        for (; i < n; i++) s += term(i);
                        S.acc[3 + lane] = s;
                    }
                    __syncthreads();
                    if (t == 0) {
                        const float cov[3][3] = {{S.acc[6], S.acc[7], S.acc[8]},
                                                 {S.acc[7], S.acc[3], S.acc[4]},
                                                 {S.acc[8], S.acc[4], S.acc[5]}};
                        float ev[3];
                        line_direction(cov, ev);
                        S.line[0] = S.acc[0]; S.line[1] = S.acc[1]; S.line[2] = S.acc[2];
                        S.line[3] = ev[0]; S.line[4] = ev[1]; S.line[5] = ev[2];
                    }
                } else if (t == 0) {
                    for (int k = 0; k < 6; k++) S.line[k] = c0[k];
                }
                __syncthreads();
                float ref[6];
                for (int k = 0; k < 6; k++) ref[k] = S.line[k];
                n_inl = select_within<NT>(ref, Q, flag, n, thr, S);
            } else if (t == 0) {
                for (int k = 0; k < 6; k++) S.line[k] = 0.f;
            }
            __syncthreads();
            SUPP_T(4);
            LineCand& out = C[j];
            if (t == 0) {
                for (int k = 0; k < 6; k++) out.line[k] = S.line[k];
                out.n_inliers = n_inl;
                out.iterations = S.iterations;
                out.idx_off = coff + used;
                int fl = 0;
                if (!((double)n_inl < sp.line_ratio * (double)bsize)) {
                    fl = 1;
                    if (line_in_range(S.line, K)) fl |= 2;
                }
                S.flags = fl;
            }
            ncand = j + 1;
            __syncthreads();
            const int fl = S.flags;
            if (!(fl & 1)) {
                if (t == 0) out.flags = fl;
                break;
            }
            int nonborder = 0;
            int wbase = 0, kbase = 0;
            for (int base = 0; base < n; base += NT) {
                const int i = base + t;
                const bool valid = i < n;
                const bool in = valid && flag[i];
                const float4 p = valid ? Q[i] : make_float4(0.f, 0.f, 0.f, 0.f);
                if (in && (fl & 2) && !is_border_point(p, D, K)) nonborder++;
                const uint64_t mi = __ballot(in), mk = __ballot(valid && !in);
                const uint64_t lt = (lane == 0) ? 0ull : (~0ull >> (64 - lane));
                if (lane == 0) { S.s0[wave] = __popcll(mi); S.s1[wave] = __popcll(mk); }
                __syncthreads();
                int oi = wbase, ok = kbase;
                for (int w = 0; w < wave; w++) { oi += S.s0[w]; ok += S.s1[w]; }
                int ti = 0, tk = 0;
                for (int w = 0; w < NT / 64; w++) { ti += S.s0[w]; tk += S.s1[w]; }
                __syncthreads();
                if (in) lidx[used + oi + __popcll(mi & lt)] = __float_as_int(p.w);
                if (valid && !in) Q[ok + __popcll(mk & lt)] = p;
                wbase += ti;
                kbase += tk;
            }
            nonborder = block_sum<NT>(nonborder, S);
            if (t == 0) out.flags = fl | ((fl & 2) && nonborder <= n_inl / 4 ? 4 : 0);
            used += n_inl;
            n = kbase;
            __syncthreads();
            SUPP_T(5);
        }
#ifdef SPSLAM_SUPP_PROF
        if (t == 0) {
            pr[7] = bsize;
            for (int k = 0; k < 8; k++) sb.prof[((size_t)f * kMaxPlanesPerFrame + q) * 8 + k] = pr[k];
        }
#endif
            return ncand;
        };
        const int ncand = in_lds ? boundary(Qs, shs, flags_s)
                                 : boundary(sb.big + (size_t)f * g.contour_cap + coff,
                                            sb.big_sh + (size_t)f * g.contour_cap + coff,
                                            sb.big_flag + (size_t)f * g.contour_cap + coff);
        if (t == 0) sb.n_cand[f * kMaxPlanesPerFrame + q] = ncand;
        __syncthreads();
    }
}

__device__ void supposed_coef(const float* ip, const float* il, float* coef) {
    const float a = fmaf(ip[1], il[5], -(ip[2] * il[4]));
    const float b = fmaf(ip[2], il[3], -(ip[0] * il[5]));
    const float c = fmaf(ip[0], il[4], -(ip[1] * il[3]));
    const float d = fmaf(c, il[2], fmaf(a, il[0], b * il[1]));
    const float v = sqrtf(fmaf(c, c, fmaf(a, a, b * b)));
    coef[0] = a / v; coef[1] = b / v; coef[2] = c / v; coef[3] = -d / v;
    if (coef[3] < 0)
        for (int k = 0; k < 4; k++) coef[k] = -coef[k];
}

__global__ __launch_bounds__(64) void supp_assemble_kernel(SuppParams sp, SuppBuffers sb, int contour_cap,
                                                           const spslam_plane* __restrict__ planes,
                                                           const int* __restrict__ plane_counts,
                                                           spslam_supposed_plane* __restrict__ out,
                                                           int* __restrict__ out_counts,
                                                           int32_t* __restrict__ out_line_idx,
                                                           float* __restrict__ out_patch) {
    __shared__ float pl[kMaxPlanesPerFrame + kMaxSuppPerFrame][4];
    __shared__ int src_cand[kMaxSuppPerFrame];
    __shared__ int n_out;
    const int f = blockIdx.x, lane = threadIdx.x;
    const int np = min(plane_counts[f], kMaxPlanesPerFrame);
    const spslam_plane* P = planes + (size_t)f * kMaxPlanesPerFrame;
    const LineCand* C = sb.cand + (size_t)f * kMaxPlanesPerFrame * kMaxLinesPerBoundary;
    spslam_supposed_plane* O = out + (size_t)f * sp.supp_cap;
    const int cap = min(sp.supp_cap, kMaxSuppPerFrame);
    const int n_patch = sp.n_steps * sp.n_steps;
    if (lane == 0) {
        for (int q = 0; q < np; q++)
            for (int k = 0; k < 4; k++) pl[q][k] = P[q].coef[k];
        int nl = np, ns = 0, loff = 0;
        for (int q = np - 1; q >= 0; --q) {
            const int nc = sb.n_cand[f * kMaxPlanesPerFrame + q];
            for (int j = 0; j < nc; j++) {
                const LineCand& c = C[q * kMaxLinesPerBoundary + j];
                if ((c.flags & 7) != 7) continue;
                float cf[4];
                supposed_coef(pl[q], c.line, cf);
                bool seen = false;
                for (int m = 0; m < nl && !seen; m++)
                    seen = plane_seen_by(pl[m], cf);
                if (seen) continue;
                if (ns < cap && nl < kMaxPlanesPerFrame + kMaxSuppPerFrame) {
                    for (int k = 0; k < 4; k++) pl[nl][k] = cf[k];
                    nl++;
                    spslam_supposed_plane& o = O[ns];
                    for (int k = 0; k < 4; k++) o.coef[k] = cf[k];
                    for (int k = 0; k < 6; k++) o.line[k] = c.line[k];
                    o.source_plane = q;
                    o.n_line = min(c.n_inliers, sp.line_cap - loff);
                    o.line_offset = loff;
                    o.n_patch = n_patch;
                    o.patch_offset = ns * n_patch;
                    o.pad = 0;
                    loff += o.n_line;
                    src_cand[ns] = q * kMaxLinesPerBoundary + j;
                }
                ns++;
            }
        }
        out_counts[f] = ns;
        n_out = min(ns, cap);
    }
    __syncthreads();
    for (int s = 0; s < n_out; s++) {
        const spslam_supposed_plane& o = O[s];
        const LineCand& c = C[src_cand[s]];
        const int32_t* src = sb.line_idx + (size_t)f * contour_cap + c.idx_off;
        int32_t* dst = out_line_idx + (size_t)f * sp.line_cap + o.line_offset;
        for (int i = lane; i < o.n_line; i += 64) dst[i] = src[i];
        const float* ip = pl[o.source_plane];
        float* pp = out_patch + ((size_t)f * sp.supp_cap + s) * (size_t)n_patch * 3;
        for (int k = lane; k < n_patch; k += 64) {
            const float a = sp.steps[k / sp.n_steps], b = sp.steps[k % sp.n_steps];
            const float x = fmaf(b, ip[0], fmaf(a, o.line[3], o.line[0]));
            const float y = fmaf(b, ip[1], fmaf(a, o.line[4], o.line[1]));
            const float z = (fmaf(o.coef[0], x, o.coef[1] * y) + o.coef[3]) / (-o.coef[2]);
            pp[3 * k] = x;
            pp[3 * k + 1] = y;
            pp[3 * k + 2] = z;
        }
    }
}

}

hipError_t supp_launch(const PlaneGeom& g, const PlaneBuffers& pb, const SuppParams& sp, const SuppBuffers& sb,
                       int n, const float* depth, long long depth_fs, int depth_stride, const spslam_plane* planes,
                       const int* plane_counts, const int32_t* contours, spslam_supposed_plane* out, int* out_counts,
                       int32_t* out_line_idx, float* out_patch, hipStream_t s, KernelTimer* timer) {
    if (sp.n_steps < 1 || sp.n_steps > kMaxPatchSteps || sp.supp_cap < 1) return hipErrorInvalidValue;
    auto B = [&](int k) { if (timer) timer->begin(k, s); };
    auto E = [&](int k) { if (timer) timer->end(k, s); };
    B(kKindSuppLines);
    if (n <= 16)
        hipLaunchKernelGGL(supp::supp_lines_kernel<512>, dim3(n, 16), dim3(512), 0, s, g, pb, sp, sb, depth,
                           depth_fs, depth_stride, planes, plane_counts, contours);
    else
        hipLaunchKernelGGL(supp::supp_lines_kernel<supp::kThreads>, dim3(n, 16), dim3(supp::kThreads), 0, s, g, pb,
                           sp, sb, depth, depth_fs, depth_stride, planes, plane_counts, contours);
    E(kKindSuppLines);
    B(kKindSuppAssemble);
    hipLaunchKernelGGL(supp::supp_assemble_kernel, dim3(n), dim3(64), 0, s, sp, sb, g.contour_cap, planes,
                       plane_counts, out, out_counts, out_line_idx, out_patch);
    E(kKindSuppAssemble);
    return hipGetLastError();
}

__global__ __launch_bounds__(64) void plane_not_seen_debug_kernel(const float* __restrict__ planes, int n,
                                                                  const float* __restrict__ coefs, int m,
                                                                  int* __restrict__ out) {
    const int k = blockIdx.x * 64 + threadIdx.x;
    if (k >= m) return;
    bool seen = false;
    for (int j = 0; j < n && !seen; j++) seen = plane_seen_by(planes + 4 * j, coefs + 4 * k);
    out[k] = !seen;
}

hipError_t plane_not_seen_debug_launch(const float* planes, int n, const float* coefs, int m, int* out,
                                       hipStream_t s) {
    if (m < 1) return hipSuccess;
    hipLaunchKernelGGL(plane_not_seen_debug_kernel, dim3((m + 63) / 64), dim3(64), 0, s, planes, n, coefs, m, out);
    return hipGetLastError();
}

}
```

### sp-slam_amd/csrc/supposed_launch.h

```cpp
#pragma once
#include <hip/hip_runtime.h>

#include "../../include/spslam_gpu.h"
#include "orb_launch.h"
#include "plane_launch.h"

namespace spslam {

constexpr int kMaxLinesPerBoundary = 4;
constexpr int kSuppRndTable = 1 << 21;
constexpr int kMaxPatchSteps = 64;
constexpr int kMaxSuppPerFrame = 32;

struct LineCand {
    float line[6];
    int n_inliers;
    int iterations;
    int flags;
    int idx_off;
};

struct SuppParams {
    double line_ratio;
    float sqr_th_f;
    float min_x, max_x, min_y, max_y;
    int supp_cap;
    int line_cap;
    int n_steps;
    float steps[kMaxPatchSteps];
};

struct SuppBuffers {
    const uint32_t* rnd;
    LineCand* cand;
    int* n_cand;
    int32_t* line_idx;
    float4* big;
    int* big_sh;
    uint8_t* big_flag;
    long long* prof;
};

hipError_t supp_launch(const PlaneGeom& g, const PlaneBuffers& pb, const SuppParams& sp, const SuppBuffers& sb,
                       int n, const float* depth, long long depth_fs, int depth_stride, const spslam_plane* planes,
                       const int* plane_counts, const int32_t* contours, spslam_supposed_plane* out, int* out_counts,
                       int32_t* out_line_idx, float* out_patch, hipStream_t s, KernelTimer* timer);

hipError_t plane_not_seen_debug_launch(const float* planes, int n, const float* coefs, int m, int* out,
                                       hipStream_t s);

}
```

### sp-slam_amd/spslam_planes.py

```python
from __future__ import annotations

import ctypes

import numpy as np

import spslam_gpu

PLANE_DTYPE = np.dtype([("coef", "<f4", 4), ("n_inliers", "<i4"), ("inlier_offset", "<i4"), ("n_contour", "<i4"),
                        ("contour_offset", "<i4")])
assert PLANE_DTYPE.itemsize == 32


class PlaneParams(ctypes.Structure):
    _fields_ = [("cloud_dis", ctypes.c_int), ("min_size", ctypes.c_int), ("angle_threshold", ctypes.c_float),
                ("distance_threshold", ctypes.c_float), ("fx", ctypes.c_float), ("fy", ctypes.c_float),
                ("cx", ctypes.c_float), ("cy", ctypes.c_float), ("width", ctypes.c_int), ("height", ctypes.c_int),
                ("line_ratio", ctypes.c_double), ("line_distance_threshold", ctypes.c_float),
                ("image_bounds", ctypes.c_float * 4)]


SUPPOSED_DTYPE = np.dtype([("coef", "<f4", 4), ("line", "<f4", 6), ("source_plane", "<i4"), ("n_line", "<i4"),
                           ("line_offset", "<i4"), ("n_patch", "<i4"), ("patch_offset", "<i4"), ("pad", "<i4")])
assert SUPPOSED_DTYPE.itemsize == 64
LINE_CAND_DTYPE = np.dtype([("line", "<f4", 6), ("n_inliers", "<i4"), ("iterations", "<i4"), ("flags", "<i4"),
                            ("idx_offset", "<i4")])


spslam_gpu.EXPORTED += ["spslam_planes_configure", "spslam_planes_capacity", "spslam_planes_extract",
                        "spslam_planes_extract_batch_device", "spslam_planes_debug", "spslam_debug_plane_labels",
                        "spslam_supposed_capacity",
                        "spslam_planes_generate_from_boundaries",
                        "spslam_planes_generate_from_boundaries_batch_device", "spslam_supposed_debug",
                        "spslam_planes_select_cloud_set",
                        "spslam_debug_plane_not_seen"]


def _bind(lib):
    vp, ip = ctypes.c_void_p, ctypes.POINTER(ctypes.c_int)
    lib.spslam_planes_configure.argtypes = [vp, ctypes.POINTER(PlaneParams)]
    lib.spslam_planes_capacity.argtypes = [vp, ip, ip, ip]
    lib.spslam_planes_extract.argtypes = [vp, vp, ctypes.c_int, ctypes.c_int, ctypes.c_int, vp, ctypes.c_int, ip, vp,
                                          vp]
    lib.spslam_planes_extract_batch_device.argtypes = [vp, vp, ctypes.c_int, ctypes.c_size_t, ctypes.c_int, vp, vp,
                                                       vp, vp, vp]
    lib.spslam_planes_debug.argtypes = [vp, ctypes.c_int, ctypes.c_int, vp, ip]
    lib.spslam_supposed_capacity.argtypes = [vp, ip, ip, ip]
    lib.spslam_planes_generate_from_boundaries.argtypes = [vp, vp, ctypes.c_int, ctypes.c_int, ctypes.c_int, vp,
                                                           ctypes.c_int, ip, vp, vp]
    lib.spslam_planes_generate_from_boundaries_batch_device.argtypes = [vp, vp, ctypes.c_int, ctypes.c_size_t,
                                                                        ctypes.c_int, vp, vp, vp, vp, vp, vp, vp, vp]
    lib.spslam_supposed_debug.argtypes = [vp, ctypes.c_int, ctypes.c_int, vp, ip, vp, ctypes.c_int]
    lib.spslam_planes_select_cloud_set.argtypes = [vp, ctypes.c_int]
    lib.spslam_debug_plane_not_seen.argtypes = [vp, vp, ctypes.c_int, vp, ctypes.c_int, vp]


def plane_not_seen(ex: spslam_gpu.OrbExtractor, planes, coefs):
    _bind(ex.lib)
    p = np.ascontiguousarray(planes, np.float32).reshape(-1, 4)
    c = np.ascontiguousarray(coefs, np.float32).reshape(-1, 4)
    out = np.zeros(max(len(c), 1), np.int32)
    ex._check(ex.lib.spslam_debug_plane_not_seen(ex.ctx, p.ctypes.data if len(p) else None, len(p),
                                                 c.ctypes.data if len(c) else None, len(c), out.ctypes.data))
    return out[:len(c)].astype(bool)


class PlaneExtractor:

    def __init__(self, ex: spslam_gpu.OrbExtractor, fx, fy, cx, cy, width=640, height=480, cloud_dis=3,
                 min_size=500, angle_threshold=3.0, distance_threshold=0.05, line_ratio=0.2,
                 line_distance_threshold=0.01, image_bounds=(0.0, 0.0, 0.0, 0.0)):
        self.ex = ex
        _bind(ex.lib)
        self.params = PlaneParams(cloud_dis, min_size, angle_threshold, distance_threshold, fx, fy, cx, cy, width,
                                  height, line_ratio, line_distance_threshold, (ctypes.c_float * 4)(*image_bounds))
        ex._check(ex.lib.spslam_planes_configure(ex.ctx, ctypes.byref(self.params)))
        pc, ic, cc = ctypes.c_int(), ctypes.c_int(), ctypes.c_int()
        ex._check(ex.lib.spslam_planes_capacity(ex.ctx, ctypes.byref(pc), ctypes.byref(ic), ctypes.byref(cc)))
        self.planes_cap, self.inlier_cap, self.contour_cap = pc.value, ic.value, cc.value
        self.W = -(-width // cloud_dis)
        self.H = -(-height // cloud_dis)
        self._supp_caps()

    def _supp_caps(self):
        a, b, c = ctypes.c_int(), ctypes.c_int(), ctypes.c_int()
        self.ex._check(self.ex.lib.spslam_supposed_capacity(self.ex.ctx, ctypes.byref(a), ctypes.byref(b),
                                                            ctypes.byref(c)))
        self.supp_cap, self.line_cap, self.patch_points = a.value, b.value, c.value

    def configure(self, **kw):
        for k, v in kw.items():
            if k == "image_bounds":
                v = (ctypes.c_float * 4)(*v)
            setattr(self.params, k, v)
        self.ex._check(self.ex.lib.spslam_planes_configure(self.ex.ctx, ctypes.byref(self.params)))
        self._supp_caps()

    def __call__(self, depth_f32: np.ndarray):
        d = np.ascontiguousarray(depth_f32, np.float32)
        planes = np.zeros(self.planes_cap, PLANE_DTYPE)
        inl = np.zeros(self.inlier_cap, np.int32)
        con = np.zeros(self.contour_cap, np.int32)
        n = ctypes.c_int()
        self.ex._check(self.ex.lib.spslam_planes_extract(self.ex.ctx, d.ctypes.data, d.shape[1], d.shape[0],
                                                         d.shape[1], planes.ctypes.data, self.planes_cap,
                                                         ctypes.byref(n), inl.ctypes.data, con.ctypes.data))
        out = dict(coef=[], inliers=[], contour=[])
        for p in planes[:n.value]:
            out["coef"].append(p["coef"].copy())
            out["inliers"].append(inl[p["inlier_offset"]:p["inlier_offset"] + p["n_inliers"]].copy())
            out["contour"].append(con[p["contour_offset"]:p["contour_offset"] + p["n_contour"]].copy())
        return out

    def extract_batch_device(self, depth_ptr, n_frames, frame_stride, stride, planes_ptr, counts_ptr, inliers_ptr,
                             contours_ptr, stream=0):
        self.ex._check(self.ex.lib.spslam_planes_extract_batch_device(
            self.ex.ctx, depth_ptr, n_frames, frame_stride, stride, planes_ptr, counts_ptr, inliers_ptr,
            contours_ptr, stream or None))

    def keep_labels(self, on=True):
        self.ex.lib.spslam_debug_plane_labels.argtypes = [ctypes.c_void_p, ctypes.c_int]
        self.ex._check(self.ex.lib.spslam_debug_plane_labels(self.ex.ctx, int(on)))

    def debug(self, frame, what):
        N = self.W * self.H
        shape, dt = {0: ((N, 3), np.float32), 1: ((N, 3), np.float32), 2: (N, np.float32), 3: (N, np.uint32)}[what]
        out = np.zeros(shape, dt)
        n = ctypes.c_int()
        self.ex._check(self.ex.lib.spslam_planes_debug(self.ex.ctx, frame, what, out.ctypes.data, ctypes.byref(n)))
        return out

    def generate_from_boundaries(self, depth_f32: np.ndarray):
        d = np.ascontiguousarray(depth_f32, np.float32)
        out = np.zeros(self.supp_cap, SUPPOSED_DTYPE)
        lines = np.zeros(self.line_cap, np.int32)
        patch = np.zeros((self.supp_cap * self.patch_points, 3), np.float32)
        n = ctypes.c_int()
        self.ex._check(self.ex.lib.spslam_planes_generate_from_boundaries(
            self.ex.ctx, d.ctypes.data, d.shape[1], d.shape[0], d.shape[1], out.ctypes.data, self.supp_cap,
            ctypes.byref(n), lines.ctypes.data, patch.ctypes.data))
        res = dict(coef=[], line=[], source=[], line_idx=[], patch=[])
        for o in out[:n.value]:
            res["coef"].append(o["coef"].copy())
            res["line"].append(o["line"].copy())
            res["source"].append(int(o["source_plane"]))
            res["line_idx"].append(lines[o["line_offset"]:o["line_offset"] + o["n_line"]].copy())
            res["patch"].append(patch[o["patch_offset"]:o["patch_offset"] + o["n_patch"]].copy())
        return res

    def select_cloud_set(self, cloud_set):
        self.ex._check(self.ex.lib.spslam_planes_select_cloud_set(self.ex.ctx, cloud_set))

    def generate_batch_device(self, depth_ptr, n_frames, frame_stride, stride, planes_ptr, counts_ptr, contours_ptr,
                              out_ptr, out_counts_ptr, line_ptr, patch_ptr, stream=0):
        self.ex._check(self.ex.lib.spslam_planes_generate_from_boundaries_batch_device(
            self.ex.ctx, depth_ptr, n_frames, frame_stride, stride, planes_ptr, counts_ptr, contours_ptr, out_ptr,
            out_counts_ptr, line_ptr, patch_ptr, stream or None))

    def line_candidates(self, frame, plane):
        cand = np.zeros(4, LINE_CAND_DTYPE)
        n = ctypes.c_int()
        idx = np.zeros(self.line_cap, np.int32)
        self.ex._check(self.ex.lib.spslam_supposed_debug(self.ex.ctx, frame, plane, cand.ctypes.data, ctypes.byref(n),
                                                         idx.ctypes.data, self.line_cap))
        out = []
        for c in cand[:n.value]:
            o = int(c["idx_offset"])
            out.append(dict(line=c["line"].copy(), n_inliers=int(c["n_inliers"]), iterations=int(c["iterations"]),
                            flags=int(c["flags"]),
                            cloud_idx=idx[o:o + c["n_inliers"]].copy() if o >= 0 else np.zeros(0, np.int32)))
        return out
```

Before: 44190.

## Precompute RANSAC sample pairs into a table and compact inliers for line fitting

Replaces the in-kernel Fisher-Yates shuffle used for RANSAC line sampling with a precomputed per-point-count table of sample pairs, built once on the host with the same RNG sequence. When the table runs out (overflow), the kernel falls back to the old shuffle path and records the fallback. The double-buffered overlap path is removed. Inliers are compacted with wave ballots before the centroid and covariance sums, so those loops cover only the inliers instead of all boundary points. The cost is a table of about 8.9 MB in device memory, plus debug hooks.

```diff
diff --git a/include/spslam_gpu.h b/include/spslam_gpu.h
--- a/include/spslam_gpu.h
+++ b/include/spslam_gpu.h
@@ -251,6 +251,11 @@
 } spslam_line_candidate;
 int spslam_supposed_debug(spslam_ctx* ctx, int frame, int plane, spslam_line_candidate* cand, int* n_cand,
                           int32_t* idx, int idx_cap);
+
+int spslam_supposed_set_sample_rows(spslam_ctx* ctx, int usable_pairs);
+
+int spslam_debug_supposed_lines(spslam_ctx* ctx, const float* xyz, int n_points, spslam_line_candidate* cand,
+                                int* n_cand, int32_t* idx, int idx_cap, int* fallbacks, int* segments);
 
 int spslam_planes_debug(spslam_ctx* ctx, int frame, int what, void* out, int* n_points);
 
diff --git a/sp-slam_amd/csrc/capi_ctx.h b/sp-slam_amd/csrc/capi_ctx.h
--- a/sp-slam_amd/csrc/capi_ctx.h
+++ b/sp-slam_amd/csrc/capi_ctx.h
@@ -156,6 +156,7 @@
     DevBuf<int32_t> d_line1;
     DevBuf<float> d_patch1;
     int supp_last_frames = 0;
+    int supp_sample_rows = kSuppSampleRow;
     bool frame_ready = false;
     FrameGeom fg{};
     DevBuf<> d_frame1;
diff --git a/sp-slam_amd/csrc/capi_planes.cpp b/sp-slam_amd/csrc/capi_planes.cpp
--- a/sp-slam_amd/csrc/capi_planes.cpp
+++ b/sp-slam_amd/csrc/capi_planes.cpp
@@ -31,17 +31,21 @@
     sp.n_steps = ns;
     const size_t F = (size_t)c->p.max_batch, CC = (size_t)g.contour_cap;
     SuppBuffers& b = c->sb;
-    const size_t bytes = (size_t)kSuppRndTable * 4 +
+    const size_t samp_n = (size_t)kSuppSampleRows * kSuppSampleRow;
+    const size_t bytes = (size_t)kSuppRndTable * 4 + samp_n * 4 +
                          F * kMaxPlanesPerFrame * kMaxLinesPerBoundary * sizeof(LineCand) +
-                         F * kMaxPlanesPerFrame * sizeof(int) + F * CC * (4 + 16 + 4 + 1) +
-                         F * kMaxPlanesPerFrame * 8 * sizeof(long long) + 9 * 256;
+                         2 * F * kMaxPlanesPerFrame * sizeof(int) + F * CC * (4 + 16 + 4 + 1) +
+                         F * kMaxPlanesPerFrame * 8 * sizeof(long long) + 11 * 256;
     hipError_t e = c->d_supp_scratch.alloc(bytes);
     if (e != hipSuccess) return e;
     uint8_t* q = c->d_supp_scratch;
     auto carve = [&](size_t n) { uint8_t* r = q; q += (n + 255) / 256 * 256; return r; };
     b.rnd = (const uint32_t*)carve((size_t)kSuppRndTable * 4);
+    b.samp = (const uint32_t*)carve(samp_n * 4);
+    b.sample_rows = c->supp_sample_rows;
     b.cand = (LineCand*)carve(F * kMaxPlanesPerFrame * kMaxLinesPerBoundary * sizeof(LineCand));
     b.n_cand = (int*)carve(F * kMaxPlanesPerFrame * sizeof(int));
+    b.n_fallback = (int*)carve(F * kMaxPlanesPerFrame * sizeof(int));
     b.line_idx = (int32_t*)carve(F * CC * 4);
     b.big = (float4*)carve(F * CC * 16);
     b.big_sh = (int*)carve(F * CC * 4);
@@ -53,6 +57,15 @@
     std::mt19937 mt(12345u);
     for (auto& v : tab) v = (uint32_t)mt() >> 1;
     e = hipMemcpy((void*)b.rnd, tab.data(), tab.size() * 4, hipMemcpyHostToDevice);
+    if (e != hipSuccess) return e;
+    static const std::vector<uint32_t> samp = [] {
+        std::vector<uint32_t> v((size_t)kSuppSampleRows * kSuppSampleRow);
+        supp_sample_table_fill(v.data());
+        return v;
+    }();
+    e = hipMemcpy((void*)b.samp, samp.data(), samp.size() * 4, hipMemcpyHostToDevice);
+    if (e != hipSuccess) return e;
+    e = hipMemset(b.n_fallback, 0, F * kMaxPlanesPerFrame * sizeof(int));
     if (e != hipSuccess) return e;
     const size_t patch = (size_t)sp.n_steps * sp.n_steps;
     if ((e = c->d_supp1.alloc(sp.supp_cap * sizeof(spslam_supposed_plane))) != hipSuccess) return e;
@@ -389,6 +402,53 @@
     return lo > idx_cap ? SPSLAM_ERR_CAPACITY : SPSLAM_OK;
 }
 
+int spslam_supposed_set_sample_rows(spslam_ctx* c, int usable_pairs) {
+    if (!c) return SPSLAM_ERR_ARG;
+    c->supp_sample_rows = std::min(std::max(usable_pairs, 0), kSuppSampleRow);
+    c->sb.sample_rows = c->supp_sample_rows;
+    return SPSLAM_OK;
+}
+
+int spslam_debug_supposed_lines(spslam_ctx* c, const float* xyz, int n_points, spslam_line_candidate* cand,
+                                int* n_cand, int32_t* idx, int idx_cap, int* fallbacks, int* segments) {
+    if (!c || !xyz || !cand || !n_cand) return SPSLAM_ERR_ARG;
+    if (!c->planes_ready) return fail(c, SPSLAM_ERR_NOT_READY, "spslam_planes_configure not called%s", "");
+    const PlaneGeom& g = c->pg;
+    if (n_points < 1 || n_points > g.N)
+        return fail(c, SPSLAM_ERR_ARG, "point list empty or longer than the organized cloud%s", "");
+    HIP_CHECK(c, hipSetDevice(c->device));
+    HIP_CHECK(c, hipDeviceSynchronize());
+    const size_t n = (size_t)n_points;
+    std::vector<float> soa(3 * n);
+    std::vector<int32_t> con(n);
+    for (size_t i = 0; i < n; i++) {
+        soa[i] = xyz[3 * i]; soa[n + i] = xyz[3 * i + 1]; soa[2 * n + i] = xyz[3 * i + 2];
+        con[i] = (int32_t)i;
+    }
+    for (int k = 0; k < 3; k++)
+        HIP_CHECK(c, hipMemcpy(c->pb.cloud + (size_t)k * g.N, soa.data() + k * n, n * 4, hipMemcpyHostToDevice));
+    c->cloud_tag[c->cloud_set] = {};
+    c->plane_last_frames = 0;
+    spslam_plane pl{};
+    pl.coef[2] = 1.f; pl.coef[3] = 1.f;
+    pl.n_contour = n_points;
+    const int one = 1;
+    HIP_CHECK(c, hipMemcpy(c->d_con1, con.data(), n * 4, hipMemcpyHostToDevice));
+    HIP_CHECK(c, hipMemcpy(c->d_planes1, &pl, sizeof pl, hipMemcpyHostToDevice));
+    HIP_CHECK(c, hipMemcpy(c->d_plane_cnt1, &one, sizeof one, hipMemcpyHostToDevice));
+    HIP_CHECK(c, hipMemsetAsync(c->d_depth_in, 0, (size_t)g.w * g.h * sizeof(float), c->stream));
+    HIP_CHECK(c, supp_launch(g, c->pb, c->sp, c->sb, 1, c->d_depth_in, (long long)g.w * g.h, g.w, c->d_planes1,
+                             c->d_plane_cnt1, c->d_con1, c->d_supp1, c->d_supp_cnt1, c->d_line1, c->d_patch1,
+                             c->stream, nullptr));
+    HIP_CHECK(c, hipStreamSynchronize(c->stream));
+    c->supp_last_frames = 1;
+    int fb = 0;
+    HIP_CHECK(c, hipMemcpy(&fb, c->sb.n_fallback, sizeof(int), hipMemcpyDeviceToHost));
+    if (fallbacks) *fallbacks = fb & 0xFFFF;
+    if (segments) *segments = fb >> 16;
+    return spslam_supposed_debug(c, 0, 0, cand, n_cand, idx, idx_cap);
+}
+
 int spslam_planes_debug(spslam_ctx* c, int frame, int what, void* out, int* n_points) {
     if (!c || !out) return SPSLAM_ERR_ARG;
     if (!c->planes_ready || frame < 0 || frame >= c->plane_last_frames)
@@ -427,6 +487,12 @@
                                kMaxPlanesPerFrame * 8 * sizeof(long long), hipMemcpyDeviceToHost));
         return SPSLAM_OK;
     }
+    if (what == 6) {
+        if (frame >= c->supp_last_frames) return fail(c, SPSLAM_ERR_NOT_READY, "no supposed-plane data for that frame%s", "");
+        HIP_CHECK(c, hipMemcpy(out, c->sb.n_fallback + (size_t)frame * kMaxPlanesPerFrame,
+                               kMaxPlanesPerFrame * sizeof(int), hipMemcpyDeviceToHost));
+        return SPSLAM_OK;
+    }
     return fail(c, SPSLAM_ERR_ARG, "unknown debug stage%s", "");
 }
 
diff --git a/sp-slam_amd/csrc/supp_sample_table.h b/sp-slam_amd/csrc/supp_sample_table.h
--- /dev/null
+++ b/sp-slam_amd/csrc/supp_sample_table.h
@@ -0,0 +1,34 @@
+#pragma once
+#include <cstddef>
+#include <cstdint>
+#include <numeric>
+#include <random>
+#include <vector>
+
+namespace spslam {
+
+constexpr int kSuppSampleMaxN = 2048;
+constexpr int kSuppSampleRow = 1088;
+constexpr int kSuppSampleRows = kSuppSampleMaxN - 1;
+
+inline size_t supp_sample_row_offset(int n, int row = kSuppSampleRow) { return (size_t)(n - 2) * row; }
+
+inline void supp_sample_table_fill(uint32_t* out, int max_n = kSuppSampleMaxN, int row = kSuppSampleRow) {
+    std::vector<uint32_t> rnd(2 * (size_t)row);
+    std::mt19937 mt(12345u);
+    for (auto& v : rnd) v = (uint32_t)mt() >> 1;
+    std::vector<uint16_t> sh((size_t)(max_n > 2 ? max_n : 2));
+    for (int n = 2; n <= max_n; n++) {
+        std::iota(sh.begin(), sh.begin() + n, (uint16_t)0);
+        uint32_t* o = out + supp_sample_row_offset(n, row);
+        for (int k = 0; k < row; k++) {
+            const uint32_t j0 = rnd[2 * (size_t)k] % (uint32_t)n;
+            const uint32_t j1 = 1u + rnd[2 * (size_t)k + 1] % (uint32_t)(n - 1);
+            uint16_t t = sh[0]; sh[0] = sh[j0]; sh[j0] = t;
+            t = sh[1]; sh[1] = sh[j1]; sh[j1] = t;
+            o[k] = (uint32_t)sh[0] | (uint32_t)sh[1] << 16;
+        }
+    }
+}
+
+}
diff --git a/sp-slam_amd/csrc/supposed_kernels.hip b/sp-slam_amd/csrc/supposed_kernels.hip
--- a/sp-slam_amd/csrc/supposed_kernels.hip
+++ b/sp-slam_amd/csrc/supposed_kernels.hip
@@ -1,4 +1,5 @@
 #include <cfloat>
+#include <type_traits>
 
 #include "libm_restated.h"
 #include "plane_not_seen.h"
@@ -7,11 +8,12 @@
 namespace spslam {
 namespace supp {
 
-constexpr int kThreads = 256, kWaves = 4;
+constexpr int kThreads = 256;
 constexpr int kMaxWaves = 8;
 constexpr int kBatch = 64;
 constexpr int kLdsPts = 2048;
 constexpr int kMaxTrials = 1001;
+static_assert(kLdsPts == kSuppSampleMaxN, "the sample table has a row for every point count held in LDS");
 
 #ifdef SPSLAM_SUPP_PROF
 #define SUPP_CLK() ((long long)__builtin_amdgcn_s_memrealtime())
@@ -23,13 +25,13 @@
 struct Shared {
     int s0[kBatch], s1[kBatch], cnt[kBatch];
     int nb, fail, done, have;
+    int ovf;
     int iterations, best, best_s0, best_s1;
     double k;
     float line[6];
     float acc[9];
     int red[kMaxWaves];
     int n_inl, flags;
-    int s0x[kBatch], s1x[kBatch], nbb[2], failb[2];
 };
 
 __device__ __forceinline__ int wave_sum(int v) {
@@ -226,12 +228,33 @@
     return block_sum<NT>(c, S);
 }
 
-#ifndef SPSLAM_SUPP_OVERLAP
-#define SPSLAM_SUPP_OVERLAP 1
-#endif
-#ifndef SPSLAM_SUPP_OVERLAP_ALL
-#define SPSLAM_SUPP_OVERLAP_ALL 0
-#endif
+template <int NT, class I>
+__device__ void compact_inliers(const uint8_t* flag, I* inl, int n, Shared& S) {
+    constexpr int NW = NT / 64;
+    const int lane = threadIdx.x & 63, wave = threadIdx.x >> 6;
+    const int per = (n + NW * 64 - 1) / (NW * 64) * 64;
+    const int b0 = wave * per, b1 = min(n, b0 + per);
+    const uint64_t lt = (lane == 0) ? 0ull : (~0ull >> (64 - lane));
+    int c = 0;
+    for (int base = b0; base < b1; base += 64) {
+        const int i = base + lane;
+        c += __popcll(__ballot(i < b1 && flag[i]));
+    }
+    __syncthreads();
+    if (lane == 0) S.red[wave] = c;
+    __syncthreads();
+    int o = 0;
+    for (int w = 0; w < wave; w++) o += S.red[w];
+    for (int base = b0; base < b1; base += 64) {
+        const int i = base + lane;
+        const bool in = i < b1 && flag[i];
+        const uint64_t m = __ballot(in);
+        if (in) inl[o + __popcll(m & lt)] = (I)i;
+        o += __popcll(m);
+    }
+    __syncthreads();
+}
+
 #ifndef SPSLAM_SUPP_MINB
 #define SPSLAM_SUPP_MINB 3
 #endif
@@ -243,13 +266,12 @@
                                                               const int* __restrict__ plane_counts,
                                                               const int32_t* __restrict__ contours) {
     __shared__ float4 Qs[kLdsPts];
-    __shared__ int shs[kLdsPts];
+    __shared__ uint16_t inl_s[kLdsPts];
     __shared__ uint8_t flags_s[kLdsPts];
 #ifdef SPSLAM_MEASURE_SKIP_SUPP
     if (g.W > 0) return;
 #endif
     __shared__ Shared S;
-    constexpr bool kOverlap = SPSLAM_SUPP_OVERLAP && (NT == 512 || SPSLAM_SUPP_OVERLAP_ALL);
     const int f = blockIdx.x, t = threadIdx.x, lane = t & 63, wave = t >> 6;
     const int np = min(plane_counts[f], kMaxPlanesPerFrame);
     const spslam_plane* P = planes + (size_t)f * kMaxPlanesPerFrame;
@@ -260,16 +282,24 @@
     const Cam K{g.fx, g.fy, g.cx, g.cy, sp.min_x, sp.max_x, sp.min_y, sp.max_y, g.w, g.h, depth_stride};
     const float* D = depth + f * depth_fs;
     const float thr = sp.sqr_th_f;
+    const int ruse = min(max(sb.sample_rows, 0), kSuppSampleRow);
+    if (blockIdx.y == 0)
+        for (int q = np + t; q < kMaxPlanesPerFrame; q += NT) sb.n_fallback[f * kMaxPlanesPerFrame + q] = 0;
     for (int q = blockIdx.y; q < np; q += gridDim.y) {
         LineCand* C = sb.cand + ((size_t)f * kMaxPlanesPerFrame + q) * kMaxLinesPerBoundary;
         const int bsize = P[q].n_contour, coff = P[q].contour_offset;
         if (bsize < 50) {
-            if (t == 0) sb.n_cand[f * kMaxPlanesPerFrame + q] = 0;
+            if (t == 0) {
+                sb.n_cand[f * kMaxPlanesPerFrame + q] = 0;
+                sb.n_fallback[f * kMaxPlanesPerFrame + q] = 0;
+            }
             continue;
         }
         const bool in_lds = bsize <= kLdsPts;
         int32_t* lidx = sb.line_idx + (size_t)f * g.contour_cap + coff;
-        auto boundary = [&](float4* Q, int* sh, uint8_t* flag) __attribute__((always_inline)) -> int {
+        int* sh = sb.big_sh + (size_t)f * g.contour_cap + coff;
+        auto boundary = [&](auto lds_tag, float4* Q, uint8_t* flag, auto* inl) __attribute__((always_inline)) -> int {
+        constexpr bool kLds = decltype(lds_tag)::value;
 #ifdef SPSLAM_SUPP_PROF
         long long pr[8] = {0, 0, 0, 0, 0, 0, 0, 0}, pt = SUPP_CLK();
 #endif
@@ -280,157 +310,55 @@
         __syncthreads();
         SUPP_T(0);
         int n = bsize, used = 0, ncand = 0;
+        int n_fb = 0, n_seg = 0;
         for (int j = 0; j < kMaxLinesPerBoundary; j++) {
-            if (t == 0) {
-                S.iterations = 0; S.best = -2147483647; S.k = 1.0; S.have = 0; S.done = n < 2;
-            }
-            if constexpr (kOverlap) {
-                if (t < kBatch) S.cnt[t] = 0;
-            }
-            for (int i = t; i < n; i += NT) sh[i] = i;
-            __syncthreads();
             const double one_over_n = 1.0 / (double)n, log_prob = log(1.0 - 0.99);
-            int r0 = 0, r1 = 1;
-            uint32_t pos = 0;
-            int bp0 = 0, bp1 = 0, qh = 0, qn = 0;
-            uint64_t gmask = 0;
-            uint32_t rnext = wave == 0 ? sb.rnd[lane] : 0u;
-            if constexpr (!kOverlap) {
-                while (!S.done) {
-                    if (wave == 0) {
-                        const int it0 = S.iterations;
-                        int nb = 0, chk = 0;
-                        bool fail = false;
-                        while (nb < kBatch && it0 + nb < kMaxTrials) {
-                            if (qh == qn) {
-                                const uint32_t r = rnext;
-                                const uint32_t jv = (lane & 1) ? 1u + r % (uint32_t)(n - 1) : r % (uint32_t)n;
-                                pos += 64;
-                                rnext = sb.rnd[pos + lane];
-    #pragma unroll 4
-                                for (int c = 0; c < 32; c++) {
-                                    const int j0 = __builtin_amdgcn_readlane((int)jv, 2 * c), j1 = __builtin_amdgcn_readlane((int)jv, 2 * c + 1);
-                                    const int i0 = j0 > 1 ? j0 : 0, i1 = j1 > 1 ? j1 : 1;
-                                    const int x0 = sh[i0], x1 = sh[i1];
-                                    const int a0 = r0, b0 = r1;
-                                    const int r1m = j0 == 1 ? a0 : b0;
-                                    sh[i0] = a0;
-                                    sh[i1] = r1m;
-                                    r0 = j0 > 1 ? x0 : (j0 == 1 ? b0 : a0);
-                                    r1 = j1 > 1 ? (j1 == j0 ? a0 : x1) : r1m;
-                                    bp0 = lane == c ? r0 : bp0;
-                                    bp1 = lane == c ? r1 : bp1;
-                                }
-                                bool good = false;
-                                if (lane < 32) {
-                                    const float4 a = Q[bp0], b = Q[bp1];
-                                    good = a.x != b.x && a.y != b.y && a.z != b.z;
-                                }
-                                gmask = __ballot(good);
-                                qh = 0;
-                                qn = 32;
-                            }
-                            const uint64_t m = gmask & (~0ull << qh) & 0xFFFFFFFFull;
-                            if (m == 0) {
-                                chk += qn - qh;
-                                qh = qn;
-                                if (chk >= 1000) { fail = true; break; }
-                                continue;
-                            }
-                            const int gi = __ffsll((unsigned long long)m) - 1;
-                            if (chk + (gi - qh) >= 1000) { fail = true; break; }
-                            const int s0v = __builtin_amdgcn_readlane(bp0, gi), s1v = __builtin_amdgcn_readlane(bp1, gi);
-                            if (lane == 0) { S.s0[nb] = s0v; S.s1[nb] = s1v; }
-                            nb++;
-                            chk = 0;
-                            qh = gi + 1;
-                        }
-                        if (lane == 0) { S.nb = nb; S.fail = fail; }
+            n_seg++;
+            for (int attempt = 0; attempt < 2; attempt++) {
+                const bool look = kLds && attempt == 0 && ruse > 0;
+                if (t == 0) {
+                    S.iterations = 0; S.best = -2147483647; S.k = 1.0; S.have = 0; S.done = n < 2; S.ovf = 0;
+                }
+                if (!look)
+                    for (int i = t; i < n; i += NT) sh[i] = i;
+                __syncthreads();
+                const uint32_t* row = sb.samp + (size_t)(max(n, 2) - 2) * kSuppSampleRow;
+                int pi = 0;
+                uint32_t nxt = (look && wave == 0) ? row[min(lane, kSuppSampleRow - 1)] : 0u;
+                auto sample_lookup = [&](int it0) __attribute__((always_inline)) {
+                    const int lim = min(kBatch, kMaxTrials - it0);
+                    const uint64_t lt = (lane == 0) ? 0ull : (~0ull >> (64 - lane));
+                    int nb = 0, chk = 0;
+                    bool fail = false, ovf = false;
+                    while (nb == 0 && lim > 0) {
+                        const int nv = min(64, ruse - pi);
+                        if (nv <= 0) { ovf = true; break; }
+                        const int a = (int)(nxt & 0xFFFFu), b = (int)(nxt >> 16);
+                        const float4 pa = Q[a], pb_ = Q[b];
+                        const bool good = lane < nv && pa.x != pb_.x && pa.y != pb_.y && pa.z != pb_.z;
+                        const uint64_t gm = __ballot(good);
+                        if (gm == 0) {
+                            chk += nv;
+                            pi += nv;
+                            if (chk >= 1000) { fail = true; break; }
+                        } else {
+                            if (chk + (__ffsll((unsigned long long)gm) - 1) >= 1000) { fail = true; break; }
+                            const int rank = __popcll(gm & lt);
+                            nb = min((int)__popcll(gm), lim);
+                            if (good && rank < nb) { S.s0[rank] = a; S.s1[rank] = b; }
+                            const uint64_t lm = __ballot(good && rank == nb - 1);
+                            pi += __ffsll((unsigned long long)lm);
+                        }
+                        nxt = row[min(pi + lane, kSuppSampleRow - 1)];
                     }
-                    __syncthreads();
-                    SUPP_T(1);
-                    const int nb = S.nb;
-                    {
-                        constexpr int NW = NT / 64;
-                        const int c = wave * (kBatch / NW) + lane / NW, qq = lane % NW;
-                        int cnt = 0;
-                        if (c < nb) {
-                            float L[6];
-                            line_from_samples(Q[S.s0[c]], Q[S.s1[c]], L);
-                            float ld[3] = {L[3], L[4], L[5]};
-                            normalize4(ld);
-    #pragma unroll 1
-                            for (int i = qq; i < n; i += NW) cnt += line_sqd(L, ld, Q[i]) <= thr;
-                        }
-    #pragma unroll
-                        for (int o = 1; o < NW; o <<= 1) cnt += __shfl_xor(cnt, o);
-                        if (qq == 0 && c < nb) S.cnt[c] = cnt;
-                    }
-                    __syncthreads();
-                    SUPP_T(2);
-                    if (wave == 0) {
-                        const int it0 = S.iterations, best0 = S.best;
-                        const double k0 = S.k;
-                        const bool act = lane < nb;
-                        const int cn = act ? S.cnt[lane] : INT_MIN;
-                        int pm = cn, lr;
-    #pragma unroll
-                        for (int off = 1; off < 64; off <<= 1) {
-                            const int y = __shfl_up(pm, off);
-                            if (lane >= off) pm = max(pm, y);
-                        }
-                        int ex = __shfl_up(pm, 1);
-                        if (lane == 0) ex = INT_MIN;
-                        const bool rec = act && cn > max(ex, best0);
-                        double kc = 0.0;
-                        if (rec) {
-                            const double w = (double)cn * one_over_n;
-                            double pno = 1.0 - w * w;
-                            pno = fmax(DBL_EPSILON, pno);
-                            pno = fmin(1.0 - DBL_EPSILON, pno);
-                            kc = log_prob / log(pno);
-                        }
-                        lr = rec ? lane : -1;
-    #pragma unroll
-                        for (int off = 1; off < 64; off <<= 1) {
-                            const int y = __shfl_up(lr, off);
-                            if (lane >= off) lr = max(lr, y);
-                        }
-                        int lre = __shfl_up(lr, 1);
-                        if (lane == 0) lre = -1;
-                        const double kb_rec = __shfl(kc, lre < 0 ? 0 : lre);
-                        const double kb = lre < 0 ? k0 : kb_rec;
-                        const uint64_t m1 = __ballot(act && !((double)(it0 + lane) < kb));
-                        const int stop1 = m1 ? __ffsll((unsigned long long)m1) - 1 : 64;
-                        const int stop2 = (kMaxTrials - 1) - it0;
-                        int proc, it;
-                        bool done;
-                        if (stop1 < nb && stop1 <= stop2) { proc = stop1; it = it0 + stop1; done = true; }
-                        else if (stop2 < nb) { proc = stop2 + 1; it = it0 + stop2 + 1; done = true; }
-                        else { proc = nb; it = it0 + nb; done = false; }
-                        const uint64_t rm = __ballot(rec) & (proc >= 64 ? ~0ull : ((1ull << proc) - 1ull));
-                        double kf = k0;
-                        if (rm) {
-                            const int L = 63 - __clzll(rm);
-                            kf = __shfl(kc, L);
-                            if (lane == L) {
-                                S.best = cn; S.best_s0 = S.s0[L]; S.best_s1 = S.s1[L]; S.have = 1; S.k = kc;
-                            }
-                        }
-                        if (!done && (S.fail || !((double)it < kf))) done = true;
-                        if (lane == 0) {
-                            S.iterations = it;
-                            S.done = done;
-                        }
-                    }
-                    __syncthreads();
-                    SUPP_T(3);
-    #ifdef SPSLAM_SUPP_PROF
-                    if (t == 0) pr[6]++;
-    #endif
-                }
-            } else {
-                auto sample = [&](int sb_, int it0) __attribute__((always_inline)) {
+                    if (lane == 0) { S.nb = nb; S.fail = fail; S.ovf = ovf; }
+                };
+                int r0 = 0, r1 = 1;
+                uint32_t pos = 0;
+                int bp0 = 0, bp1 = 0, qh = 0, qn = 0;
+                uint64_t gmask = 0;
+                uint32_t rnext = (!look && wave == 0) ? sb.rnd[lane] : 0u;
+                auto sample_replay = [&](int it0) __attribute__((always_inline)) {
                     int nb = 0, chk = 0;
                     bool fail = false;
                     while (nb < kBatch && it0 + nb < kMaxTrials) {
@@ -439,7 +367,7 @@
                             const uint32_t jv = (lane & 1) ? 1u + r % (uint32_t)(n - 1) : r % (uint32_t)n;
                             pos += 64;
                             rnext = sb.rnd[pos + lane];
-    #pragma unroll 4
+#pragma unroll 4
                             for (int c = 0; c < 32; c++) {
                                 const int j0 = __builtin_amdgcn_readlane((int)jv, 2 * c), j1 = __builtin_amdgcn_readlane((int)jv, 2 * c + 1);
                                 const int i0 = j0 > 1 ? j0 : 0, i1 = j1 > 1 ? j1 : 1;
@@ -472,105 +400,104 @@
                         const int gi = __ffsll((unsigned long long)m) - 1;
                         if (chk + (gi - qh) >= 1000) { fail = true; break; }
                         const int s0v = __builtin_amdgcn_readlane(bp0, gi), s1v = __builtin_amdgcn_readlane(bp1, gi);
-                        if (lane == 0) { (sb_ ? S.s0x : S.s0)[nb] = s0v; (sb_ ? S.s1x : S.s1)[nb] = s1v; }
+                        if (lane == 0) { S.s0[nb] = s0v; S.s1[nb] = s1v; }
                         nb++;
                         chk = 0;
                         qh = gi + 1;
                     }
-                    if (lane == 0) { S.nbb[sb_] = nb; S.failb[sb_] = fail; }
+                    if (lane == 0) { S.nb = nb; S.fail = fail; }
                 };
-                auto decide = [&](int sb_, int nb) __attribute__((always_inline)) {
-                    const int it0 = S.iterations, best0 = S.best;
-                    const double k0 = S.k;
-                    const bool act = lane < nb;
-                    const int cn = act ? S.cnt[lane] : INT_MIN;
-                    int pm = cn, lr;
-    #pragma unroll
-                    for (int off = 1; off < 64; off <<= 1) {
-                        const int y = __shfl_up(pm, off);
-                        if (lane >= off) pm = max(pm, y);
+                while (!S.done) {
+                    if (wave == 0) {
+                        if (look) sample_lookup(S.iterations);
+                        else sample_replay(S.iterations);
                     }
-                    int ex = __shfl_up(pm, 1);
-                    if (lane == 0) ex = INT_MIN;
-                    const bool rec = act && cn > max(ex, best0);
-                    double kc = 0.0;
-                    if (rec) {
-                        const double w = (double)cn * one_over_n;
-                        double pno = 1.0 - w * w;
-                        pno = fmax(DBL_EPSILON, pno);
-                        pno = fmin(1.0 - DBL_EPSILON, pno);
-                        kc = log_prob / log(pno);
-                    }
-                    lr = rec ? lane : -1;
-    #pragma unroll
-                    for (int off = 1; off < 64; off <<= 1) {
-                        const int y = __shfl_up(lr, off);
-                        if (lane >= off) lr = max(lr, y);
-                    }
-                    int lre = __shfl_up(lr, 1);
-                    if (lane == 0) lre = -1;
-                    const double kb_rec = __shfl(kc, lre < 0 ? 0 : lre);
-                    const double kb = lre < 0 ? k0 : kb_rec;
-                    const uint64_t m1 = __ballot(act && !((double)(it0 + lane) < kb));
-                    const int stop1 = m1 ? __ffsll((unsigned long long)m1) - 1 : 64;
-                    const int stop2 = (kMaxTrials - 1) - it0;
-                    int proc, it;
-                    bool done;
-                    if (stop1 < nb && stop1 <= stop2) { proc = stop1; it = it0 + stop1; done = true; }
-                    else if (stop2 < nb) { proc = stop2 + 1; it = it0 + stop2 + 1; done = true; }
-                    else { proc = nb; it = it0 + nb; done = false; }
-                    const uint64_t rm = __ballot(rec) & (proc >= 64 ? ~0ull : ((1ull << proc) - 1ull));
-                    double kf = k0;
-                    if (rm) {
-                        const int L = 63 - __clzll(rm);
-                        kf = __shfl(kc, L);
-                        if (lane == L) {
-                            S.best = cn; S.best_s0 = (sb_ ? S.s0x : S.s0)[L]; S.best_s1 = (sb_ ? S.s1x : S.s1)[L];
-                            S.have = 1; S.k = kc;
-                        }
-                    }
-                    if (!done && (S.failb[sb_] || !((double)it < kf))) done = true;
-                    if (lane == 0) {
-                        S.iterations = it;
-                        S.done = done;
-                    }
-                };
-                if (wave == 0 && !S.done) sample(0, 0);
-                __syncthreads();
-                SUPP_T(1);
-                int cur = 0;
-                while (!S.done) {
-                    const int nb = S.nbb[cur];
-                    if (wave == 0) {
-                        if (!S.failb[cur]) sample(cur ^ 1, S.iterations + nb);
-                        else if (lane == 0) { S.nbb[cur ^ 1] = 0; S.failb[cur ^ 1] = 1; }
-                    } else {
-                        constexpr int LP = NT / 64 - 1;
-                        const int u = t - 64, c = u / LP, qq = u - c * LP;
+                    __syncthreads();
+                    SUPP_T(1);
+                    if (S.ovf) break;
+                    const int nb = S.nb;
+                    {
+                        constexpr int NW = NT / 64;
+                        const int c = wave * (kBatch / NW) + lane / NW, qq = lane % NW;
+                        int cnt = 0;
                         if (c < nb) {
                             float L[6];
-                            line_from_samples(Q[(cur ? S.s0x : S.s0)[c]], Q[(cur ? S.s1x : S.s1)[c]], L);
+                            line_from_samples(Q[S.s0[c]], Q[S.s1[c]], L);
                             float ld[3] = {L[3], L[4], L[5]};
                             normalize4(ld);
-                            int cnt = 0;
 #pragma unroll 1
-                            for (int i = qq; i < n; i += LP) cnt += line_sqd(L, ld, Q[i]) <= thr;
-                            atomicAdd(&S.cnt[c], cnt);
-                        }
+                            for (int i = qq; i < n; i += NW) cnt += line_sqd(L, ld, Q[i]) <= thr;
+                        }
+#pragma unroll
+                        for (int o = 1; o < NW; o <<= 1) cnt += __shfl_xor(cnt, o);
+                        if (qq == 0 && c < nb) S.cnt[c] = cnt;
                     }
                     __syncthreads();
                     SUPP_T(2);
                     if (wave == 0) {
-                        decide(cur, nb);
-                        S.cnt[lane] = 0;
+                        const int it0 = S.iterations, best0 = S.best;
+                        const double k0 = S.k;
+                        const bool act = lane < nb;
+                        const int cn = act ? S.cnt[lane] : INT_MIN;
+                        int pm = cn, lr;
+#pragma unroll
+                        for (int off = 1; off < 64; off <<= 1) {
+                            const int y = __shfl_up(pm, off);
+                            if (lane >= off) pm = max(pm, y);
+                        }
+                        int ex = __shfl_up(pm, 1);
+                        if (lane == 0) ex = INT_MIN;
+                        const bool rec = act && cn > max(ex, best0);
+                        double kc = 0.0;
+                        if (rec) {
+                            const double w = (double)cn * one_over_n;
+                            double pno = 1.0 - w * w;
+                            pno = fmax(DBL_EPSILON, pno);
+                            pno = fmin(1.0 - DBL_EPSILON, pno);
+                            kc = log_prob / log(pno);
+                        }
+                        lr = rec ? lane : -1;
+#pragma unroll
+                        for (int off = 1; off < 64; off <<= 1) {
+                            const int y = __shfl_up(lr, off);
+                            if (lane >= off) lr = max(lr, y);
+                        }
+                        int lre = __shfl_up(lr, 1);
+                        if (lane == 0) lre = -1;
+                        const double kb_rec = __shfl(kc, lre < 0 ? 0 : lre);
+                        const double kb = lre < 0 ? k0 : kb_rec;
+                        const uint64_t m1 = __ballot(act && !((double)(it0 + lane) < kb));
+                        const int stop1 = m1 ? __ffsll((unsigned long long)m1) - 1 : 64;
+                        const int stop2 = (kMaxTrials - 1) - it0;
+                        int proc, it;
+                        bool done;
+                        if (stop1 < nb && stop1 <= stop2) { proc = stop1; it = it0 + stop1; done = true; }
+                        else if (stop2 < nb) { proc = stop2 + 1; it = it0 + stop2 + 1; done = true; }
+                        else { proc = nb; it = it0 + nb; done = false; }
+                        const uint64_t rm = __ballot(rec) & (proc >= 64 ? ~0ull : ((1ull << proc) - 1ull));
+                        double kf = k0;
+                        if (rm) {
+                            const int L = 63 - __clzll(rm);
+                            kf = __shfl(kc, L);
+                            if (lane == L) {
+                                S.best = cn; S.best_s0 = S.s0[L]; S.best_s1 = S.s1[L]; S.have = 1; S.k = kc;
+                            }
+                        }
+                        if (!done && (S.fail || !((double)it < kf))) done = true;
+                        if (lane == 0) {
+                            S.iterations = it;
+                            S.done = done;
+                        }
                     }
                     __syncthreads();
                     SUPP_T(3);
 #ifdef SPSLAM_SUPP_PROF
                     if (t == 0) pr[6]++;
 #endif
-                    cur ^= 1;
                 }
+                if (!S.ovf) break;
+                n_fb++;
+                __syncthreads();
             }
             int n_inl = 0;
             if (S.have) {
@@ -578,46 +505,45 @@
                 line_from_samples(Q[S.best_s0], Q[S.best_s1], c0);
                 n_inl = select_within<NT>(c0, Q, flag, n, thr, S);
                 if (n_inl > 2) {
+                    compact_inliers<NT>(flag, inl, n, S);
                     constexpr int kG = 8;
                     if (wave == 0 && lane < 3) {
+                        auto term = [&](int i) __attribute__((always_inline)) {
+                            const float4 p = Q[inl[i]];
+                            return lane == 0 ? p.x : lane == 1 ? p.y : p.z;
+                        };
                         float s = 0.f;
                         int i = 0;
-                        for (; i + kG <= n; i += kG) {
+                        for (; i + kG <= n_inl; i += kG) {
                             float v[kG];
 #pragma unroll
-                            for (int u = 0; u < kG; u++) {
-                                const float4 p = Q[i + u];
-                                v[u] = flag[i + u] ? (lane == 0 ? p.x : lane == 1 ? p.y : p.z) : 0.f;
-                            }
+                            for (int u = 0; u < kG; u++) v[u] = term(i + u);
 #pragma unroll
                             for (int u = 0; u < kG; u++) s += v[u];
                         }
-                        for (; i < n; i++) {
-                            const float4 p = Q[i];
-                            s += flag[i] ? (lane == 0 ? p.x : lane == 1 ? p.y : p.z) : 0.f;
-                        }
+                        for (; i < n_inl; i++) s += term(i);
                         S.acc[lane] = s / (float)n_inl;
                     }
                     __syncthreads();
                     if (wave == 0 && lane < 6) {
                         const float cx = S.acc[0], cy = S.acc[1], cz = S.acc[2];
                         auto term = [&](int i) __attribute__((always_inline)) {
-                            const float4 p = Q[i];
+                            const float4 p = Q[inl[i]];
                             const float x = p.x - cx, y = p.y - cy, z = p.z - cz;
                             const float a = lane == 0 ? y : lane == 1 ? y : lane == 2 ? z : lane == 3 ? x : lane == 4 ? y : z;
                             const float b = lane == 0 ? y : lane == 1 ? z : lane == 2 ? z : x;
-                            return flag[i] ? a * b : 0.f;
+                            return a * b;
                         };
                         float s = 0.f;
                         int i = 0;
-                        for (; i + kG <= n; i += kG) {
+                        for (; i + kG <= n_inl; i += kG) {
                             float v[kG];
 #pragma unroll
                             for (int u = 0; u < kG; u++) v[u] = term(i + u);
 #pragma unroll
                             for (int u = 0; u < kG; u++) s += v[u];
                         }
-                        for (; i < n; i++) s += term(i);
+                        for (; i < n_inl; i++) s += term(i);
                         S.acc[3 + lane] = s;
                     }
                     __syncthreads();
@@ -697,12 +623,12 @@
             for (int k = 0; k < 8; k++) sb.prof[((size_t)f * kMaxPlanesPerFrame + q) * 8 + k] = pr[k];
         }
 #endif
+            if (t == 0) sb.n_fallback[f * kMaxPlanesPerFrame + q] = n_fb | (n_seg << 16);
             return ncand;
         };
-        const int ncand = in_lds ? boundary(Qs, shs, flags_s)
-                                 : boundary(sb.big + (size_t)f * g.contour_cap + coff,
-                                            sb.big_sh + (size_t)f * g.contour_cap + coff,
-                                            sb.big_flag + (size_t)f * g.contour_cap + coff);
+        const int ncand = in_lds ? boundary(std::true_type{}, Qs, flags_s, inl_s)
+                                 : boundary(std::false_type{}, sb.big + (size_t)f * g.contour_cap + coff,
+                                            sb.big_flag + (size_t)f * g.contour_cap + coff, sh);
         if (t == 0) sb.n_cand[f * kMaxPlanesPerFrame + q] = ncand;
         __syncthreads();
     }
diff --git a/sp-slam_amd/csrc/supposed_launch.h b/sp-slam_amd/csrc/supposed_launch.h
--- a/sp-slam_amd/csrc/supposed_launch.h
+++ b/sp-slam_amd/csrc/supposed_launch.h
@@ -4,6 +4,7 @@
 #include "../../include/spslam_gpu.h"
 #include "orb_launch.h"
 #include "plane_launch.h"
+#include "supp_sample_table.h"
 
 namespace spslam {
 
@@ -32,8 +33,11 @@
 
 struct SuppBuffers {
     const uint32_t* rnd;
+    const uint32_t* samp;
+    int sample_rows;
     LineCand* cand;
     int* n_cand;
+    int* n_fallback;
     int32_t* line_idx;
     float4* big;
     int* big_sh;
diff --git a/sp-slam_amd/spslam_planes.py b/sp-slam_amd/spslam_planes.py
--- a/sp-slam_amd/spslam_planes.py
+++ b/sp-slam_amd/spslam_planes.py
@@ -32,7 +32,8 @@
                         "spslam_planes_generate_from_boundaries",
                         "spslam_planes_generate_from_boundaries_batch_device", "spslam_supposed_debug",
                         "spslam_planes_select_cloud_set",
-                        "spslam_debug_plane_not_seen"]
+                        "spslam_debug_plane_not_seen", "spslam_supposed_set_sample_rows",
+                        "spslam_debug_supposed_lines"]
 
 
 def _bind(lib):
@@ -156,14 +157,40 @@
             self.ex.ctx, depth_ptr, n_frames, frame_stride, stride, planes_ptr, counts_ptr, contours_ptr, out_ptr,
             out_counts_ptr, line_ptr, patch_ptr, stream or None))
 
+    def set_sample_rows(self, usable_pairs=1 << 30):
+        self.ex.lib.spslam_supposed_set_sample_rows.argtypes = [ctypes.c_void_p, ctypes.c_int]
+        self.ex._check(self.ex.lib.spslam_supposed_set_sample_rows(self.ex.ctx, int(usable_pairs)))
+
+    def sampler_fallbacks(self, frame):
+        buf = np.zeros(self.planes_cap, np.int32)
+        n = ctypes.c_int()
+        self.ex._check(self.ex.lib.spslam_planes_debug(self.ex.ctx, frame, 6, buf.ctypes.data, ctypes.byref(n)))
+        return int((buf & 0xFFFF).sum()), int((buf >> 16).sum())
+
+    def debug_lines(self, xyz):
+        p = np.ascontiguousarray(xyz, np.float32).reshape(-1, 3)
+        cand = np.zeros(4, LINE_CAND_DTYPE)
+        n, fb, seg = ctypes.c_int(), ctypes.c_int(), ctypes.c_int()
+        idx = np.zeros(self.line_cap, np.int32)
+        vp, ip = ctypes.c_void_p, ctypes.POINTER(ctypes.c_int)
+        self.ex.lib.spslam_debug_supposed_lines.argtypes = [vp, vp, ctypes.c_int, vp, ip, vp, ctypes.c_int, ip, ip]
+        self.ex._check(self.ex.lib.spslam_debug_supposed_lines(
+            self.ex.ctx, p.ctypes.data, len(p), cand.ctypes.data, ctypes.byref(n), idx.ctypes.data, self.line_cap,
+            ctypes.byref(fb), ctypes.byref(seg)))
+        return self._candidates(cand[:n.value], idx), fb.value, seg.value
+
     def line_candidates(self, frame, plane):
         cand = np.zeros(4, LINE_CAND_DTYPE)
         n = ctypes.c_int()
         idx = np.zeros(self.line_cap, np.int32)
         self.ex._check(self.ex.lib.spslam_supposed_debug(self.ex.ctx, frame, plane, cand.ctypes.data, ctypes.byref(n),
                                                          idx.ctypes.data, self.line_cap))
+        return self._candidates(cand[:n.value], idx)
+
+    @staticmethod
+    def _candidates(cand, idx):
         out = []
-        for c in cand[:n.value]:
+        for c in cand:
             o = int(c["idx_offset"])
             out.append(dict(line=c["line"].copy(), n_inliers=int(c["n_inliers"]), iterations=int(c["iterations"]),
                             flags=int(c["flags"]),
```

After: 44630 (median of 6 runs). No clear change (+1.0%).
